# Xinglab/lr2rmats

Hardware: AMD Instinct MI355X
Metric: long-read alignments classified/sec; achieved HBM GB/s vs roofline (higher is better)
Workload: dtype int32

## Files before the change

lr2rmats_amd/csrc/l2r_engine.hip:

```cpp
#include <hip/hip_runtime.h>
#include <stdarg.h>
#include <stdio.h>
#include <stdlib.h>
#include <string.h>
#include <algorithm>
#include <initializer_list>
#include <string>
#include <type_traits>
#include <utility>
#include <vector>

#include "../../include/lr2rmats_hip.h"
#include "l2r_kernels.hip.h"
#include "l2r_window.hip.h"
#include "l2r_slab.hip.h"
#include "l2r_chunk.hip.h"
#include "l2r_tchunk.hip.h"
#include "l2r_filter.hip.h"
#include "l2r_fusion.hip.h"
#include "l2r_sj.hip.h"
#include "l2r_sort.hip.h"
#include "l2r_names.hip.h"
#include "l2r_gtf.hip.h"
#include "l2r_bed.hip.h"
#include "l2r_uniq.hip.h"
#include "l2r_plan.hip.h"
#include "l2r_tables.hip.h"
#include "l2r_nameorder.hip.h"
#include "l2r_gtforder.hip.h"
#include "l2r_bedplan.hip.h"

using namespace l2r;

static thread_local char g_err[1024] = "";

static int fail(int code, const char *fmt, ...)
{
    va_list ap;
    va_start(ap, fmt);
    vsnprintf(g_err, sizeof g_err, fmt, ap);
    va_end(ap);
    return code;
}

#define HIP_TRY(expr)                                                                                   \
    do {                                                                                                \
        hipError_t e_ = (expr);                                                                         \
        if (e_ != hipSuccess) return fail(-2, "[%s] %s: %s", __func__, #expr, hipGetErrorString(e_));   \
    } while (0)

template <typename T>
struct DevBuf {
    T *p = nullptr;
    size_t cap = 0;
    DevBuf() = default;
    DevBuf(const DevBuf &) = delete;
    DevBuf &operator=(const DevBuf &) = delete;
    ~DevBuf() { release(); }
    int ensure(size_t n)
    {
        if (n <= cap && p) return 0;
        if (p) { (void)hipFree(p); p = nullptr; cap = 0; }
        const size_t want = n ? n : 1;
        T *q = nullptr;
        const hipError_t e = hipMalloc((void **)&q, want * sizeof(T));
        if (e != hipSuccess) return fail(-2, "hipMalloc(%zu bytes): %s", want * sizeof(T), hipGetErrorString(e));
        p = q; cap = want;
        return 0;
    }
    void release() { if (p) (void)hipFree(p); p = nullptr; cap = 0; }
};

struct EventPair {
    hipEvent_t a = nullptr, b = nullptr;
    EventPair() = default;
    EventPair(const EventPair &) = delete;
    EventPair &operator=(const EventPair &) = delete;
    ~EventPair() { if (a) (void)hipEventDestroy(a); if (b) (void)hipEventDestroy(b); }
};

struct StageTimer {
    bool on = false, wait = false;
    hipEvent_t ev[2] = {nullptr, nullptr};
    StageTimer() = default;
    StageTimer(const StageTimer &) = delete;
    StageTimer &operator=(const StageTimer &) = delete;
    ~StageTimer() { for (int k = 0; k < 2; ++k) if (ev[k]) (void)hipEventDestroy(ev[k]); }
    int begin(bool on_, bool wait_)
    {
        on = on_; wait = wait_;
        for (int k = 0; k < 2 && on; ++k) if (!ev[k]) HIP_TRY(hipEventCreate(&ev[k]));
        return 0;
    }
    template <typename F> int launch(l2r_ctx *c, double *ms, F f);
};

enum class Pipeline { classic, slab, tile };

struct SjRowBuf {
    DevBuf<int32_t> col[6];
    size_t cap = 0;
    SjCols cols() const { return SjCols{col[0].p, col[1].p, col[2].p, col[3].p, col[4].p, col[5].p}; }
};
struct SjState {
    bool open = false, finished = false;
    bool over = false;
    SjPrm prm{3, 1};
    int32_t n_seq = 0;
    DevBuf<int64_t> seq_off; DevBuf<uint8_t> bases;
    SjRowBuf rows[2]; int cur = 0;
    int64_t n_rows = 0;
    int64_t compact_rows = (int64_t)1 << 24, compact_at = (int64_t)1 << 24;
    DevBuf<uint16_t> flag; DevBuf<int32_t> tid, pos; DevBuf<uint8_t> uniq; DevBuf<int64_t> cig_off; DevBuf<uint32_t> cig, cnt;
    DevBuf<uint32_t> hist12, tile_hist, head, word;
    DevBuf<uint8_t> strand[2], motif[2], anno[2]; int bcur = 0;
    DevBuf<int32_t> near_acc;
    double stats[32] = {0};
    StageTimer clk;
};
struct SjIntrons {
    DevBuf<int32_t> tx_tid, ex_start, ex_end; DevBuf<int64_t> tx_ex_off;
    SjState st;
};

struct SortState {
    DevBuf<uint16_t> flag; DevBuf<int32_t> tid, pos;
    DevBuf<uint64_t> key[2]; DevBuf<uint32_t> idx[2];
    DevBuf<uint32_t> hist, tile_hist, word;
    StageTimer clk;
    double stats[7] = {0};
};

struct NameState {
    DevBuf<uint64_t> blob, hkey;
    DevBuf<int64_t> off;
    DevBuf<uint32_t> head, head_pos, first_idx, sizes, order;
    DevBuf<uint32_t> word;
    StageTimer clk;
    double stats[11] = {0};
};

struct GtfState {
    DevBuf<uint4> text;
    DevBuf<uint32_t> tile_cnt, start;
    DevBuf<uint32_t> kept, tx, l_name_off, l_name_len, l_s, l_e;
    DevBuf<uint32_t> r_start, r_len, r_line, r_tx;
    DevBuf<uint32_t> t_name_off, t_name_len, t_s, t_e, head;
    DevBuf<uint32_t> h_off, h_len, rank;
    DevBuf<uint32_t> c, s, e, order1, order;
    DevBuf<uint32_t> word;
    std::vector<uint64_t> res_start; std::vector<uint32_t> res_len, res_line;
    StageTimer clk;
    double stats[17] = {0};
};

struct BedState {
    bool begun = false;
    l2r_bed_params prm{};
    std::vector<int64_t> h_ref_off; std::vector<uint8_t> h_ref_names;
    DevBuf<int64_t> ref_off; DevBuf<uint8_t> ref_names;
    DevBuf<uint16_t> flag; DevBuf<int32_t> tid, pos; DevBuf<uint8_t> mapq, names; DevBuf<int64_t> cig_off, name_off; DevBuf<uint32_t> cig;
    DevBuf<uint32_t> off, n_blocks, span, size_len;
    DevBuf<uint32_t> word;
    DevBuf<uint4> text;
    bool have_text = false, text_on_host = false;
    int64_t n_bytes = 0;
    std::vector<uint8_t> host_text;
    StageTimer clk;
    double stats[11] = {0};
};

struct UniqState {
    DevBuf<int32_t> tid, xs, xe; DevBuf<uint8_t> rev; DevBuf<int64_t> ex_off;
    DevBuf<UniqRec> rec; DevBuf<uint64_t> tile_max;
    DevBuf<uint32_t> head, first, len, word;
    DevBuf<int32_t> l_src, l_start, l_end, l_cov;
    DevBuf<int32_t> uniq_of, u_src, u_start, u_end, u_cov; DevBuf<uint8_t> merged;
    bool have = false, on_host = false;
    int64_t n = 0, n_unique = 0;
    UniqResult host;
    StageTimer clk;
    double stats[UQS_N] = {0};
};

struct RunFacts {
    bool known = false;
    uint32_t n_wide = 0;
    uint32_t n_chunk = 0;
    uint32_t n_rest = 0;
    uint32_t n_late = 0;
    uint32_t n_fb = 0;
    uint32_t n_wide_rest = 0;
    unsigned long long chunk_rest = 0;
    bool redo_empty = false;
};

struct l2r_ctx {
    int device = 0;
    hipStream_t stream = nullptr;
    hipStream_t side[2] = {nullptr, nullptr};
    hipEvent_t ev_fork = nullptr, ev_join[2] = {nullptr, nullptr};

    int fast_grid = 0;
    int n_cu = 256, wg_per_cu = 4;
    int ablate = 0;
    int64_t seg_max = SEG_MAX;
    Pipeline want_pipe = Pipeline::tile;
    bool pipeline_forced = false;
    bool wide_direct = true;
    bool chunk_direct = true;
    bool tile_split = true;
    bool side_on = true;
    bool env_tile_anyway = false, env_launch_all = false;
    bool check_stages = false;
    bool env_stamps = false;
    int64_t tile_resident = 0;
    bool tile_starved = false;
    int64_t n_lb_fallback = 0;

    l2r_params prm;
    std::string anno_cache_dir;
    int anno_cache_state = 0;
    unsigned want = L2R_WANT_RESULTS | L2R_WANT_ACCEPTED;
    bool one_shot_upload = false;

    bool sorted = true;
    int reads_per_tile = TILE_THREADS;
    int64_t n_tiles = 0, n_tiles256 = 0;
    bool wide_cigar = false;
    bool many_exon_reads = false;
    bool slab_ok = false;
    bool have_index = false;
    float index_ms = 0.0f;
    DevBuf<SlotRec> slot_rec;
    DevBuf<TileStat> tile_stat; std::vector<TileStat> h_tile_stat;
    DevBuf<TileStat> sup_stat;
    DevBuf<uint16_t> sum_nn;
    DevBuf<uint32_t> tile_sbase, s_pre, s_loc, s_pl, cig_off32, tile_rec, tile_total, tile_xbase, tile_span;
    DevBuf<int32_t> dense_start, dense_end;
    DevBuf<uint32_t> slab_row;
    DevBuf<TileWin> tw;
    DevBuf<TileWin64> tw64; DevBuf<uint32_t> wide_list, chunk_list, list_cnt, tile_flags;
    DevBuf<unsigned long long> ovf_cursor;
    DevBuf<unsigned long long> lb_tile, lb_blk, lb_sup;
    DevBuf<uint32_t> fb_list;
    DevBuf<uint32_t> rest_list;

    Pipeline pipe = Pipeline::classic;
    bool prev_run_tile = false;
    uint32_t lc_flip = 0;
    uint32_t lb_flip = 0;
    RunFacts facts;
    int64_t inexact_tiles = -1;
    int64_t n_tx = 0, n_anno_exon = 0;
    DevBuf<TxHdr> hdr;
    DevBuf<int2> anno_ex;
    DevBuf<int64_t> anno_key;
    DevBuf<SiteEnt> sk_st, sk_en;
    DevBuf<uint32_t> sd_st, sd_en, sr_st;
    DevBuf<int32_t> tid_base; int32_t n_tid_dir = 0;
    DevBuf<uint32_t> key_dir; DevBuf<int32_t> kb_base; int32_t n_tid_key = 0;
    DevBuf<int32_t> j0;
    int64_t n_compact = 0, n_wide = 0;
    std::vector<int64_t> h_anno_key_raw;
    std::vector<int64_t> h_anno_key_pm;
    int64_t n_sj = 0;
    DevBuf<int32_t> sj_tid, sj_don, sj_acc, sj_uniq, sj_multi;
    DevBuf<int64_t> sj_key;
    DevBuf<int32_t> sj_cbase, sj_dbase; DevBuf<uint32_t> sj_cdir, sj_ddir; DevBuf<int4> sj_row; int32_t sj_ntid = 0;
    std::vector<int64_t> h_sj_key_raw;
    std::vector<int64_t> h_sj_key_pm;
    int64_t n_reads = 0, n_cigar = 0, first_read = 0;
    DevBuf<int32_t> r_tid, r_pos;
    DevBuf<uint8_t> r_rev;
    DevBuf<int64_t> cig_off;
    DevBuf<uint32_t> cig;
    std::vector<int32_t> h_tid, h_pos;
    struct Stream {
        bool valid = false, sorted = true;
        int64_t next = 0;
        int64_t last_key = INT64_MIN;
        int64_t anno_cur = 0, sj_cur = 0;
        int64_t anno_cur_start = 0, sj_cur_start = 0;
        bool sj_pending = false;
    } seq;
    DevBuf<int32_t> win_start, sj_cursor;
    bool have_win = false;
    DevBuf<uint32_t> local, tile_base, ex_off, info, tile_acc, tile_acc_ex, tile_acc_at, tile_acc_ex_at, tile_chunk, tile_rchunk, totals;
    DevBuf<uint32_t> redo;
    DevBuf<uint8_t> order;
    DevBuf<TileDesc> desc;
    DevBuf<int2> walked;
    DevBuf<uint32_t> tile_first;
    DevBuf<TxHdr> win_hdr;
    DevBuf<int32_t> ex_start, ex_end, ref_tx;
    DevBuf<uint8_t> ex_flag;
    int64_t ex_cap = 0;
    DevBuf<AccRec> acc_rec;
    DevBuf<uint32_t> acc_ex_off;
    DevBuf<int32_t> acc_start, acc_end;
    DevBuf<uint8_t> acc_flag;
    bool ran = false;
    DevBuf<unsigned long long> stamps;
    uint32_t h_totals[3] = {0, 0, 0};
    bool totals_valid = false;
    SjState sj;
    SjIntrons sj_intr;
    double fusion_stats[5] = {0, 0, 0, 0, 0};
    StageTimer fusion_clk;
    SortState sort;
    NameState name;
    GtfState gtf;
    BedState bed;
    UniqState uniq;
};

template <typename F> int StageTimer::launch(l2r_ctx *c, double *ms, F f)
{
    if (on) HIP_TRY(hipEventRecord(ev[0], c->stream));
    f();
    HIP_TRY(hipGetLastError());
    if (on) {
        float t = 0.0f;
        HIP_TRY(hipEventRecord(ev[1], c->stream));
        HIP_TRY(hipEventSynchronize(ev[1]));
        HIP_TRY(hipEventElapsedTime(&t, ev[0], ev[1]));
        *ms += t;
    }
    if (wait) HIP_TRY(hipStreamSynchronize(c->stream));
    return 0;
}

static void forget_list_state(l2r_ctx *c)
{
    c->facts = RunFacts{};
    c->inexact_tiles = -1;
}

static bool lists_empty(const RunFacts &f) { return f.n_fb == 0u && f.n_wide == 0u && f.n_chunk == 0u && f.n_late == 0u; }
static bool lists_heavy(const l2r_ctx *c)
{
    const RunFacts &f = c->facts;
    return 2ull * ((unsigned long long)f.n_fb + (c->wide_direct ? f.n_wide_rest : f.n_wide) + f.chunk_rest) > (unsigned long long)c->n_tiles;
}
static bool list_runs(const l2r_ctx *c, unsigned long long n) { return !c->facts.known || n != 0ull || c->env_launch_all; }
static unsigned list_grid(const l2r_ctx *c, uint32_t n) { return c->facts.known ? std::max(n, 1u) : (unsigned)std::max<int64_t>(c->n_tiles, 1); }

static uint32_t *lc_this_run(const l2r_ctx *c) { return c->list_cnt.p + LC_WORDS * (c->lc_flip & 1u); }
static uint32_t *lc_next_run(const l2r_ctx *c) { return c->list_cnt.p + LC_WORDS * ((c->lc_flip & 1u) ^ 1u); }
static uint32_t *lc_last_run(const l2r_ctx *c) { return lc_next_run(c); }
static hipError_t lc_reset(l2r_ctx *c) { c->lc_flip = 0; return hipMemsetAsync(c->list_cnt.p, 0, 2 * LC_WORDS * sizeof(uint32_t), c->stream); }
static void end_of_run(l2r_ctx *c, bool tile) { if (tile) { c->lb_flip ^= 1u; c->lc_flip ^= 1u; } c->prev_run_tile = tile; }

static DevParams dev_params(const l2r_ctx *c)
{
    DevParams p;
    p.min_exon = c->prm.min_exon; p.min_intron = c->prm.min_intron; p.max_delet = c->prm.max_delet;
    p.ss_dis = c->prm.ss_dis; p.full_level = c->prm.full_level; p.use_multi = c->prm.use_multi;
    p.min_sj_cnt = c->prm.min_sj_cnt; p.split_trans = c->prm.split_trans; p.frac = c->prm.single_exon_ovlp_frac;
    p.n_tx = (int32_t)c->n_tx; p.n_sj = (int32_t)c->n_sj; p.reads_per_tile = c->reads_per_tile;
    p.ablate = c->ablate; p.want = (int32_t)c->want;
    if (c->n_sj > 0 && (c->ablate & (512 | 1024))) p.ablate |= 2;
    return p;
}

template <typename F> static void with_level(int level, F &&f)
{
    switch (level) {
    case 1: f(std::integral_constant<int, 1>()); break;
    case 2: f(std::integral_constant<int, 2>()); break;
    case 3: f(std::integral_constant<int, 3>()); break;
    case 4: f(std::integral_constant<int, 4>()); break;
    case 5: f(std::integral_constant<int, 5>()); break;
    default: f(std::integral_constant<int, 0>()); break;
    }
}
template <typename F> static void with_flag(bool on, F &&f)
{
    if (on) f(std::true_type());
    else f(std::false_type());
}

template <bool WIDE, bool EXACT>
static void launch_k_tile(const l2r_ctx *c, const DevParams &p, const SlabArgs &sa, unsigned grid, hipStream_t st)
{
    with_level(p.full_level, [&](auto L) { with_flag(p.ss_dis > 0, [&](auto D) { with_flag(!WIDE && (c->want & L2R_WANT_ACCEPTED), [&](auto A) {
        if constexpr (!(WIDE && A))
            hipLaunchKernelGGL(HIP_KERNEL_NAME(k_tile<L, A, D, WIDE, EXACT>), dim3(grid), dim3(TILE_THREADS), 0, st, sa, (const TileRec *)c->tile_rec.p, (const TileWin *)c->tw.p,
                               (const TileStat *)c->tile_stat.p, (const SlotRec *)c->slot_rec.p, c->tile_xbase.p);
    }); }); });
}

template <typename T> static int to_dev(l2r_ctx *c, DevBuf<T> &b, const T *src, size_t n)
{
    if (b.ensure(n ? n : 1)) return -2;
    if (n) HIP_TRY(hipMemcpyAsync(b.p, src, n * sizeof(T), hipMemcpyHostToDevice, c->stream));
    return 0;
}
template <typename T> static int put_dev(l2r_ctx *c, DevBuf<T> &b, const std::vector<T> &v) { return to_dev(c, b, v.data(), v.size()); }

extern "C" {

int l2r_abi_version(void) { return L2R_ABI_VERSION; }
const char *l2r_last_error(void) { return g_err; }

int l2r_device_count(void)
{
    int n = 0;
    if (hipGetDeviceCount(&n) != hipSuccess) return 0;
    return n;
}

l2r_ctx *l2r_create(int device)
{
    int n = 0;
    hipError_t e = hipGetDeviceCount(&n);
    if (e != hipSuccess || n <= 0) { fail(-1, "[l2r_create] no HIP device available (%s); this library has no CPU path", hipGetErrorString(e)); return nullptr; }
    if (device < 0 || device >= n) { fail(-1, "[l2r_create] device %d out of range (have %d)", device, n); return nullptr; }
    if ((e = hipSetDevice(device)) != hipSuccess) { fail(-2, "[l2r_create] hipSetDevice: %s", hipGetErrorString(e)); return nullptr; }
    l2r_ctx *c = new l2r_ctx();
    c->device = device;
    if ((e = hipStreamCreateWithFlags(&c->stream, hipStreamNonBlocking)) != hipSuccess) {
        fail(-2, "[l2r_create] hipStreamCreate: %s", hipGetErrorString(e)); delete c; return nullptr;
    }
    int prio_lo = 0, prio_hi = 0;
    (void)hipDeviceGetStreamPriorityRange(&prio_lo, &prio_hi);
    for (int k = 0; k < 2; ++k)
        if (((e = hipStreamCreateWithPriority(&c->side[k], hipStreamNonBlocking, prio_hi)) != hipSuccess &&
             ((void)hipGetLastError(), e = hipStreamCreateWithFlags(&c->side[k], hipStreamNonBlocking)) != hipSuccess) ||
            (e = hipEventCreateWithFlags(&c->ev_join[k], hipEventDisableTiming)) != hipSuccess) {
            fail(-2, "[l2r_create] side stream: %s", hipGetErrorString(e)); l2r_destroy(c); return nullptr;
        }
    if ((e = hipEventCreateWithFlags(&c->ev_fork, hipEventDisableTiming)) != hipSuccess) { fail(-2, "[l2r_create] hipEventCreate: %s", hipGetErrorString(e)); l2r_destroy(c); return nullptr; }
    c->prm = l2r_params{3, 3, 50, 0, 0x7fffffff, 5, 0, 0, 1, 0, 0.80f};
    {
        hipDeviceProp_t prop;
        if (hipGetDeviceProperties(&prop, device) == hipSuccess && prop.multiProcessorCount > 0) c->n_cu = prop.multiProcessorCount;
        const char *e = getenv("L2R_WG_PER_CU");
        if (e && atoi(e) > 0) c->wg_per_cu = atoi(e);
        e = getenv("L2R_FAST_GRID");
        if (e && atoi(e) > 0) c->fast_grid = atoi(e);
        e = getenv("L2R_ABLATE");
        c->ablate = e ? atoi(e) : 0;
        c->check_stages = getenv("L2R_CHECK") != nullptr;
        e = getenv("L2R_SEG_MAX");
        if (e && atoll(e) >= 0) c->seg_max = atoll(e);
        e = getenv("L2R_ANNO_CACHE");
        if (e && *e) c->anno_cache_dir = e;
        e = getenv("L2R_WIDE_DIRECT");
        if (e) c->wide_direct = atoi(e) != 0;
        c->env_tile_anyway = getenv("L2R_TILE_ANYWAY") != nullptr; c->env_launch_all = getenv("L2R_LAUNCH_ALL") != nullptr;
        e = getenv("L2R_CHUNK_DIRECT");
        if (e) c->chunk_direct = atoi(e) != 0;
        e = getenv("L2R_TILE_SPLIT");
        if (e) c->tile_split = atoi(e) != 0;
        e = getenv("L2R_SIDE");
        if (e) c->side_on = atoi(e) != 0;
        c->env_stamps = getenv("L2R_STAMPS") != nullptr;
        e = getenv("L2R_PIPELINE");
        if (e) { c->want_pipe = !strcmp(e, "classic") ? Pipeline::classic : !strcmp(e, "slab") ? Pipeline::slab : Pipeline::tile; c->pipeline_forced = true; }
        {
            int per_cu = 0;
            if (hipOccupancyMaxActiveBlocksPerMultiprocessor(&per_cu, k_tile<3, false, false, false>, TILE_THREADS, 0) != hipSuccess) { (void)hipGetLastError(); per_cu = 0; }
            c->tile_resident = (int64_t)per_cu * c->n_cu;
            if ((int64_t)per_cu * c->n_cu < 8 * (int64_t)TILE_GROUP + 1 || getenv("L2R_TILE_STARVED")) c->tile_starved = true;
        }
    }
    return c;
}

void l2r_destroy(l2r_ctx *c)
{
    if (!c) return;
    (void)hipSetDevice(c->device);
    for (int k = 0; k < 2; ++k) { if (c->side[k]) (void)hipStreamDestroy(c->side[k]); if (c->ev_join[k]) (void)hipEventDestroy(c->ev_join[k]); }
    if (c->ev_fork) (void)hipEventDestroy(c->ev_fork);
    if (c->stream) (void)hipStreamDestroy(c->stream);
    delete c;
}

void *l2r_stream(l2r_ctx *c) { return c ? (void *)c->stream : nullptr; }
float l2r_upload_index_ms(l2r_ctx *c) { return c ? c->index_ms : 0.0f; }
int l2r_hint_single_run(l2r_ctx *c, int on) { if (!c) return fail(-1, "[l2r_hint_single_run] null context"); c->one_shot_upload = on != 0; return 0; }

int l2r_set_outputs(l2r_ctx *c, unsigned want)
{
    if (!c) return fail(-1, "[l2r_set_outputs] null context");
    if (!(want & (L2R_WANT_RESULTS | L2R_WANT_ACCEPTED)) || (want & ~(unsigned)(L2R_WANT_RESULTS | L2R_WANT_ACCEPTED)))
        return fail(-1, "[l2r_set_outputs] want = %u: expected L2R_WANT_RESULTS and/or L2R_WANT_ACCEPTED", want);
    c->want = want;
    c->ran = false; forget_list_state(c);
    return 0;
}

int l2r_set_params(l2r_ctx *c, const l2r_params *prm)
{
    if (!c || !prm) return fail(-1, "[l2r_set_params] null argument");
    c->prm = *prm;
    c->ran = false; forget_list_state(c);
    return 0;
}

int l2r_set_annotation_cache(l2r_ctx *c, const char *dir)
{
    if (!c) return fail(-1, "[l2r_set_annotation_cache] null context");
    c->anno_cache_dir = dir ? dir : "";
    return 0;
}

int l2r_annotation_cache_state(l2r_ctx *c) { return c ? c->anno_cache_state : -1; }

int l2r_set_annotation(l2r_ctx *c, const l2r_annotation *a)
{
    if (!c || !a) return fail(-1, "[l2r_set_annotation] null argument");
    if (a->n_tx < 0 || a->n_tx > 0x7ffffff0LL || a->n_exon < 0 || a->n_exon > 0x7ffffff0LL) return fail(-1, "[l2r_set_annotation] size out of range");
    HIP_TRY(hipSetDevice(c->device));
    AnnoTables t;
    std::string msg;
    c->anno_cache_state = 0;
    const int state = anno_tables(a, c->anno_cache_dir, t, msg);
    if (state < 0) return fail(-1, "%s", msg.c_str());
    c->anno_cache_state = state;
    int rc = 0;
    if ((rc = put_dev(c, c->sk_st, t.st_ent)) || (rc = put_dev(c, c->sd_st, t.st_dir)) || (rc = put_dev(c, c->sr_st, t.st_rdir)) ||
        (rc = put_dev(c, c->sk_en, t.en_ent)) || (rc = put_dev(c, c->sd_en, t.en_dir)) || (rc = put_dev(c, c->tid_base, t.tid_base)) ||
        (rc = put_dev(c, c->key_dir, t.key_dir)) || (rc = put_dev(c, c->kb_base, t.kb_base)) || (rc = put_dev(c, c->hdr, t.hdr)) ||
        (rc = put_dev(c, c->anno_key, t.key)) || (rc = put_dev(c, c->anno_ex, t.ex))) return rc;
    HIP_TRY(hipStreamSynchronize(c->stream));
    c->h_anno_key_raw.swap(t.key_raw);
    c->h_anno_key_pm.swap(t.key);
    c->seq = l2r_ctx::Stream();
    c->n_compact = t.n_compact; c->n_wide = t.n_wide; c->n_tid_dir = t.n_tid_dir; c->n_tid_key = t.n_tid_key;
    c->n_tx = a->n_tx; c->n_anno_exon = a->n_exon;
    c->have_win = false; c->ran = false; forget_list_state(c);
    return 0;
}

int l2r_set_junctions(l2r_ctx *c, const l2r_junctions *s)
{
    if (!c) return fail(-1, "[l2r_set_junctions] null context");
    HIP_TRY(hipSetDevice(c->device));
    c->ran = false; forget_list_state(c);
    if (!s || s->n == 0) { c->n_sj = 0; c->h_sj_key_raw.clear(); c->h_sj_key_pm.clear(); c->seq = l2r_ctx::Stream(); return 0; }
    SjTables t;
    std::string msg;
    if (build_sj_tables(s, t, msg)) return fail(-1, "%s", msg.c_str());
    const size_t n = (size_t)s->n;
    int rc = 0;
    if ((rc = put_dev(c, c->sj_row, t.row)) || (rc = put_dev(c, c->sj_cbase, t.cbase)) || (rc = put_dev(c, c->sj_cdir, t.cdir)) ||
        (rc = put_dev(c, c->sj_dbase, t.dbase)) || (rc = put_dev(c, c->sj_ddir, t.ddir)) ||
        (rc = to_dev(c, c->sj_tid, s->tid, n)) || (rc = to_dev(c, c->sj_don, s->don, n)) || (rc = to_dev(c, c->sj_acc, s->acc, n)) ||
        (rc = to_dev(c, c->sj_uniq, s->uniq_c, n)) || (rc = to_dev(c, c->sj_multi, s->multi_c, n)) || (rc = put_dev(c, c->sj_key, t.key))) return rc;
    HIP_TRY(hipStreamSynchronize(c->stream));
    c->sj_ntid = t.n_tid;
    c->n_sj = s->n;
    c->h_sj_key_raw.swap(t.key_raw);
    c->h_sj_key_pm.swap(t.key);
    c->seq = l2r_ctx::Stream();
    return 0;
}

static int prepare_unsorted_windows(l2r_ctx *c);
static int finish_stream_sj_cursor(l2r_ctx *c);

static int stream_begin_upload(l2r_ctx *c, const l2r_reads *r)
{
    l2r_ctx::Stream &st = c->seq;
    const bool cont = st.valid && r->first_read_index > 0 && r->first_read_index == st.next;
    if (cont) { int rc = finish_stream_sj_cursor(c); if (rc) return rc; }
    else st = l2r_ctx::Stream();
    st.anno_cur_start = st.anno_cur; st.sj_cur_start = st.sj_cur;
    st.next = r->first_read_index + r->n_reads; st.valid = true;
    st.sj_pending = false;
    return 0;
}

static int stage_reads(l2r_ctx *c, const l2r_reads *r, const UploadPlan &pl)
{
    const int64_t N = r->n_reads;
    if (c->tile_first.ensure(pl.tile_first.size())) return -2;
    HIP_TRY(hipMemcpyAsync(c->tile_first.p, pl.tile_first.data(), pl.tile_first.size() * 4, hipMemcpyHostToDevice, c->stream));
    if (c->r_tid.ensure((size_t)N) || c->r_pos.ensure((size_t)N) || c->r_rev.ensure((size_t)N) ||
        c->cig_off.ensure((size_t)N + 1) || c->cig.ensure((size_t)r->n_cigar + 8)) return -2;
    if (N) {
        HIP_TRY(hipMemcpyAsync(c->r_tid.p, r->tid, (size_t)N * 4, hipMemcpyHostToDevice, c->stream));
        HIP_TRY(hipMemcpyAsync(c->r_pos.p, r->pos, (size_t)N * 4, hipMemcpyHostToDevice, c->stream));
        HIP_TRY(hipMemcpyAsync(c->r_rev.p, r->rev, (size_t)N, hipMemcpyHostToDevice, c->stream));
        HIP_TRY(hipMemcpyAsync(c->cig_off.p, r->cig_off, (size_t)(N + 1) * 8, hipMemcpyHostToDevice, c->stream));
        if (r->n_cigar) HIP_TRY(hipMemcpyAsync(c->cig.p, r->cig, (size_t)r->n_cigar * 4, hipMemcpyHostToDevice, c->stream));
    }
    return 0;
}

static int count_exon_bound(l2r_ctx *c, const l2r_reads *r, bool wide_cigar, size_t *exb)
{
    *exb = (size_t)r->n_cigar + (size_t)r->n_reads;
    if (!wide_cigar) return 0;
    if (c->totals.ensure(TOT_WORDS)) return -2;
    unsigned long long *d_cnt = reinterpret_cast<unsigned long long *>(c->totals.p);
    HIP_TRY(hipMemsetAsync(d_cnt, 0, 8, c->stream));
    hipLaunchKernelGGL(k_count_cut_ops, dim3(4096), dim3(TILE_THREADS), 0, c->stream, (const uint32_t *)c->cig.p, (int64_t)r->n_cigar, d_cnt);
    unsigned long long cuts = 0;
    HIP_TRY(hipMemcpyAsync(&cuts, d_cnt, 8, hipMemcpyDeviceToHost, c->stream));
    HIP_TRY(hipStreamSynchronize(c->stream));
    *exb = (size_t)cuts + (size_t)r->n_reads;
    return 0;
}

static int reserve_work(l2r_ctx *c, size_t n_reads, size_t exb)
{
    const size_t N = n_reads, T = (size_t)c->n_tiles;
    if (c->j0.ensure(N) || c->local.ensure(N + 1) || c->ex_off.ensure(N) || c->info.ensure(N) || c->ref_tx.ensure(N) ||
        c->redo.ensure(N) || c->order.ensure(N + TILE_THREADS) || c->desc.ensure(T) || c->win_hdr.ensure(T * WIN_TX) ||
        c->tile_base.ensure(T + 1) || c->tile_acc.ensure(T + 1) || c->tile_acc_ex.ensure(T + 1) ||
        c->tile_acc_at.ensure(T + 2) || c->tile_acc_ex_at.ensure(T + 2) ||
        c->totals.ensure(TOT_WORDS) || c->tile_chunk.ensure(T + 1) || c->tile_rchunk.ensure(T + 1) || c->ex_start.ensure(exb) || c->ex_end.ensure(exb) || c->ex_flag.ensure(exb) ||
        c->acc_rec.ensure(N) || c->acc_ex_off.ensure(N) ||
        c->acc_start.ensure(exb) || c->acc_end.ensure(exb) || c->acc_flag.ensure(exb) || (c->wide_cigar && c->walked.ensure((T + 1) * LDS_EXON_CAP))) return -2;
    c->ex_cap = (int64_t)exb;
    return 0;
}

static int stage_slab(l2r_ctx *c, size_t n_reads, const UploadPlan &pl)
{
    const size_t N = n_reads, T = (size_t)pl.n_tiles;
    if (c->tw64.ensure(T + 1) || c->wide_list.ensure(2 * (T + 1)) || c->chunk_list.ensure(2 * (T + 1)) || c->list_cnt.ensure(2 * LC_WORDS) || c->tile_flags.ensure(T + 8) ||
        c->lb_tile.ensure(T + 64) || c->lb_blk.ensure(T / LB_BLK + 64) || c->lb_sup.ensure(2 * ((T >> LB_SUP_SHIFT) + 64)) || c->fb_list.ensure(T + 1) || c->rest_list.ensure(T + 1) || c->tile_stat.ensure(T + 1) || c->sup_stat.ensure((T >> LB_SUP_SHIFT) + 2) ||
        (!c->wide_cigar && c->slot_rec.ensure((T + 1) * TILE_THREADS))) return -2;
    HIP_TRY(hipMemsetAsync(c->lb_sup.p, 0, 2 * ((T >> LB_SUP_SHIFT) + 64) * 8, c->stream)); c->lb_flip = 0;
    HIP_TRY(lc_reset(c)); c->prev_run_tile = false;
    if (c->tile_sbase.ensure(T + 1) || c->ovf_cursor.ensure(1) || c->tw.ensure(T + 1) || c->tile_total.ensure(T + 2) || c->tile_xbase.ensure(T + 2) || c->tile_span.ensure(12 * (T + 1)) ||
        c->s_pre.ensure(N + 1) || c->s_loc.ensure(N + 1) ||
        c->slab_row.ensure((size_t)pl.slab_total + 4) ||
        c->dense_start.ensure((size_t)pl.dense_rows + 1) || c->dense_end.ensure((size_t)pl.dense_rows + 1)) return -2;
    HIP_TRY(hipMemsetAsync(c->ovf_cursor.p, 0, 8, c->stream));
    HIP_TRY(hipMemcpyAsync(c->tile_sbase.p, pl.sbase.data(), (T + 1) * 4, hipMemcpyHostToDevice, c->stream));
    if (c->tile_rec.ensure(8 * (T + 1)) || c->cig_off32.ensure(N + 2) || c->s_pl.ensure(N + 1)) return -2;
    HIP_TRY(hipMemcpyAsync(c->tile_rec.p, pl.rec.data(), pl.rec.size() * sizeof(TileRec), hipMemcpyHostToDevice, c->stream));
    HIP_TRY(hipMemcpyAsync(c->cig_off32.p, pl.off32.data(), pl.off32.size() * 4, hipMemcpyHostToDevice, c->stream));
    return 0;
}

static int make_tile_index(l2r_ctx *c, const l2r_reads *r, const UploadPlan &pl)
{
    const size_t N = (size_t)r->n_reads, T = (size_t)pl.n_tiles;
    const bool summaries = r->cig_summary != nullptr;
    c->h_tile_stat = pl.tile_stat;
    c->index_ms = 0.0f; c->have_index = pl.have_index;
    if (!pl.have_index) return 0;
    EventPair ev;
    HIP_TRY(hipEventCreate(&ev.a)); HIP_TRY(hipEventCreate(&ev.b));
    if (summaries) {
        if (c->sum_nn.ensure(N + 1)) return -2;
        HIP_TRY(hipMemcpyAsync(c->sum_nn.p, pl.nn.data(), N * 2, hipMemcpyHostToDevice, c->stream));
        HIP_TRY(hipMemcpyAsync(c->tile_stat.p, c->h_tile_stat.data(), T * sizeof(TileStat), hipMemcpyHostToDevice, c->stream));
    }
    const unsigned gi = (unsigned)std::min<size_t>(T, 8192);
    HIP_TRY(hipEventRecord(ev.a, c->stream));
    with_flag(summaries, [&](auto S) {
        hipLaunchKernelGGL(HIP_KERNEL_NAME(k_tile_index<S>), dim3(gi), dim3(TILE_THREADS), 0, c->stream, (TileRec *)c->tile_rec.p, c->tile_stat.p, c->slot_rec.p, (uint32_t)T,
                           (const uint32_t *)c->cig_off32.p, (const int32_t *)c->r_pos.p, (const uint8_t *)c->r_rev.p, (const uint32_t *)c->cig.p, S ? (const uint16_t *)c->sum_nn.p : (const uint16_t *)nullptr);
    });
    HIP_TRY(hipEventRecord(ev.b, c->stream));
    if (!summaries) {
        HIP_TRY(hipMemcpyAsync(c->h_tile_stat.data(), c->tile_stat.p, T * sizeof(TileStat), hipMemcpyDeviceToHost, c->stream));
        HIP_TRY(hipStreamSynchronize(c->stream));
    }
    HIP_TRY(hipEventSynchronize(ev.b));
    HIP_TRY(hipEventElapsedTime(&c->index_ms, ev.a, ev.b));
    return 0;
}

int l2r_upload_reads(l2r_ctx *c, const l2r_reads *r)
{
    if (!c || !r) return fail(-1, "[l2r_upload_reads] null argument");
    if (r->n_reads < 0 || r->n_cigar < 0) return fail(-1, "[l2r_upload_reads] negative size");
    if ((uint64_t)r->n_cigar + (uint64_t)r->n_reads >= 0xfffffff0ULL)
        return fail(-1, "[l2r_upload_reads] shard too large for 32-bit exon offsets (%lld ops + %lld reads); split it", (long long)r->n_cigar, (long long)r->n_reads);
    HIP_TRY(hipSetDevice(c->device));
    const int64_t N = r->n_reads;
    UploadPlan pl;
    std::vector<TileStat> sup;
    struct Drain { hipStream_t s; ~Drain() { (void)hipStreamSynchronize(s); } } drain{c->stream};
    std::string msg;
    if (int rc = plan_check_reads(*r, pl, msg)) return fail(rc, "%s", msg.c_str());

    if (int rc = stream_begin_upload(c, r)) return rc;

    PlanOpts po;
    po.min_intron = c->prm.min_intron; po.max_delet = c->prm.max_delet;
    po.want_slab = c->want_pipe != Pipeline::classic;
    po.want_index = c->want_pipe == Pipeline::tile && !(c->one_shot_upload && !c->env_tile_anyway && !c->pipeline_forced);
    po.stream_sorted = c->seq.sorted; po.last_key = c->seq.last_key;
    plan_tiles(*r, po, pl);
    c->seq.sorted = pl.sorted; c->seq.last_key = pl.last_key;
    const bool sorted = pl.sorted;
    c->sorted = sorted; c->have_win = false;
    if (!sorted || c->n_sj > 0) { c->h_tid.assign(r->tid, r->tid + N); c->h_pos.assign(r->pos, r->pos + N); }
    else { c->h_tid.clear(); c->h_pos.clear(); }
    c->wide_cigar = pl.wide_cigar; c->many_exon_reads = pl.many_exon_reads;
    c->reads_per_tile = pl.reads_per_tile; c->n_tiles = pl.n_tiles; c->n_tiles256 = pl.n_tiles256;

    if (int rc = stage_reads(c, r, pl)) return rc;
    size_t exb = 0;
    if (int rc = count_exon_bound(c, r, pl.wide_cigar, &exb)) return rc;
    if (int rc = reserve_work(c, (size_t)N, exb)) return rc;

    plan_slab(*r, exb, pl);
    c->slab_ok = pl.slab_ok; c->pipe = Pipeline::classic;
    if (pl.slab_ok) {
        if (int rc = stage_slab(c, (size_t)N, pl)) return rc;
        if (int rc = make_tile_index(c, r, pl)) return rc;
        sup = plan_sup_stat(pl, c->h_tile_stat);
        HIP_TRY(hipMemcpyAsync(c->sup_stat.p, sup.data(), sup.size() * sizeof(TileStat), hipMemcpyHostToDevice, c->stream));
    }
    if (c->env_stamps && !c->stamps.p) {
        if (c->stamps.ensure(1024 * 8 + 16)) return -2;
        HIP_TRY(hipMemsetAsync(c->stamps.p, 0, (1024 * 8 + 16) * 8, c->stream));
    }
    HIP_TRY(hipStreamSynchronize(c->stream));

    c->n_reads = N; c->n_cigar = r->n_cigar; c->first_read = r->first_read_index;
    c->ran = false; c->totals_valid = false; forget_list_state(c);
    if (sorted) {
        if (N) c->seq.anno_cur = std::max(c->seq.anno_cur, cursor_after(c->h_anno_key_pm, r->tid[N - 1], r->pos[N - 1]));
        c->seq.sj_pending = c->n_sj > 0;
    } else {
        int rc = prepare_unsorted_windows(c);
        if (rc) return rc;
    }
    return 0;
}

static int finish_stream_sj_cursor(l2r_ctx *c)
{
    l2r_ctx::Stream &st = c->seq;
    if (!st.sj_pending || !c->ran || c->n_sj == 0 || c->n_reads == 0) { st.sj_pending = false; return 0; }
    const int64_t N = c->n_reads;
    std::vector<uint32_t> info((size_t)N);
    HIP_TRY(hipMemcpyAsync(info.data(), c->info.p, (size_t)N * 4, hipMemcpyDeviceToHost, c->stream));
    HIP_TRY(hipStreamSynchronize(c->stream));
    for (int64_t i = N - 1; i >= 0; --i) {
        if ((info[(size_t)i] & (I_FULL | I_KNOWN | I_KSITE)) != (I_FULL | I_KSITE)) continue;
        st.sj_cur = std::max(st.sj_cur, cursor_after(c->h_sj_key_pm, c->h_tid[(size_t)i], c->h_pos[(size_t)i]));
        break;
    }
    st.sj_pending = false;
    return 0;
}

static int prepare_unsorted_windows(l2r_ctx *c)
{
    if (c->sorted || c->have_win) return 0;
    const int64_t N = c->n_reads;
    std::vector<int32_t> w((size_t)N);
    c->seq.anno_cur = cursor_replay(c->h_anno_key_raw, c->seq.anno_cur_start, c->h_tid.data(), c->h_pos.data(), N, w.data(), [](int64_t) { return true; });
    if (c->win_start.ensure((size_t)N)) return -2;
    if (N) HIP_TRY(hipMemcpyAsync(c->win_start.p, w.data(), (size_t)N * 4, hipMemcpyHostToDevice, c->stream));
    HIP_TRY(hipStreamSynchronize(c->stream));
    c->have_win = true;
    return 0;
}

static int prepare_unsorted_sj_cursor(l2r_ctx *c)
{
    const int64_t N = c->n_reads;
    std::vector<uint32_t> info((size_t)N);
    if (N) HIP_TRY(hipMemcpyAsync(info.data(), c->info.p, (size_t)N * 4, hipMemcpyDeviceToHost, c->stream));
    HIP_TRY(hipStreamSynchronize(c->stream));
    std::vector<int32_t> cur_v((size_t)N);
    c->seq.sj_cur = cursor_replay(c->h_sj_key_raw, c->seq.sj_cur_start, c->h_tid.data(), c->h_pos.data(), N, cur_v.data(),
                                  [&](int64_t i) { return (info[(size_t)i] & (I_FULL | I_KNOWN | I_KSITE)) == (I_FULL | I_KSITE); });
    if (c->sj_cursor.ensure((size_t)N)) return -2;
    if (N) HIP_TRY(hipMemcpyAsync(c->sj_cursor.p, cur_v.data(), (size_t)N * 4, hipMemcpyHostToDevice, c->stream));
    HIP_TRY(hipStreamSynchronize(c->stream));
    return 0;
}

enum { ST_PASS_A = 0, ST_SCAN1, ST_FAST, ST_GENERIC, ST_SJ, ST_SCAN2, ST_GATHER, ST_N };

static Pipeline choose_pipeline(l2r_ctx *c, const DevParams &p)
{
    if (!(c->slab_ok && p.min_intron >= 0 && p.min_intron < (1 << 28) && p.max_delet >= -1 && p.max_delet < (1 << 28) - 1 &&
          (!c->wide_cigar || p.min_exon >= 1)))
        return Pipeline::classic;
    if (c->want_pipe != Pipeline::tile || c->wide_cigar || p.min_exon < 1 || !(c->have_index || c->n_tiles == 0) || c->tile_starved)
        return Pipeline::slab;
    if (c->inexact_tiles < 0) {
        int64_t inexact = 0;
        for (const TileStat &st : c->h_tile_stat) inexact += tile_exact(st, p.min_exon, p.min_intron, p.max_delet) ? 0 : 1;
        c->inexact_tiles = inexact;
    }
    if (c->inexact_tiles * 50 > c->n_tiles + 800 && !c->env_tile_anyway) return Pipeline::slab;
    if (c->facts.known && lists_heavy(c) && !c->env_tile_anyway) return Pipeline::slab;
    return Pipeline::tile;
}

static const char *const stage_name[ST_N + 1] = {"(start)", "pass A / order", "scan / walk", "classification", "generic", "junction check", "accepted scan", "accepted gather"};
#define MARK(i) do { if (ev) HIP_TRY(hipEventRecord(ev[i], c->stream)); \
        if (c->check_stages) { const hipError_t e_ = hipStreamSynchronize(c->stream); \
            if (e_ != hipSuccess) return fail(-2, "[launch_all] device error behind stage \"%s\": %s", stage_name[i], hipGetErrorString(e_)); } } while (0)

static FastArgs fast_args(const l2r_ctx *c, const DevParams &p, const SiteTabs &tabs, const int32_t *j0)
{
    FastArgs fa;
    fa.n_reads = c->n_reads; fa.r_tid = c->r_tid.p; fa.r_pos = c->r_pos.p; fa.r_rev = c->r_rev.p; fa.cig_off = c->cig_off.p; fa.cig = c->cig.p;
    fa.walked = c->walked.p; fa.local = c->local.p; fa.order = c->order.p; fa.tile_base = c->tile_base.p; fa.j0 = j0; fa.desc = c->desc.p; fa.win_hdr = c->win_hdr.p;
    fa.hdr = c->hdr.p; fa.st = tabs.st; fa.en = tabs.en;
    fa.ex_off = c->ex_off.p; fa.ex_start = c->ex_start.p; fa.ex_end = c->ex_end.p; fa.ex_flag = c->ex_flag.p; fa.info = c->info.p; fa.ref_tx = c->ref_tx.p;
    fa.tile_acc = c->tile_acc.p; fa.tile_acc_ex = c->tile_acc_ex.p; fa.redo_count = c->totals.p + TOT_REDO; fa.redo = c->redo.p;
    fa.tile_chunk = c->tile_chunk.p; fa.tile_rchunk = c->tile_rchunk.p; fa.chunk_cursor = (unsigned long long *)(c->totals.p + TOT_CHUNK_CURSOR);
    fa.acc_start = c->acc_start.p; fa.acc_end = c->acc_end.p; fa.acc_flag = c->acc_flag.p; fa.acc_rec = (AccRec *)c->acc_rec.p; fa.acc_ex_off = c->acc_ex_off.p; fa.first_read = c->first_read;
    fa.stamps = c->stamps.p; fa.p = p;
    return fa;
}

static bool split_wait_free(const l2r_ctx *c) { return c->inexact_tiles == 0 && !(c->ablate & 256); }
static uint32_t split_mode(const l2r_ctx *c)
{
    if (!c->tile_split || !c->rest_list.p) return SPLIT_OFF;
    const uint32_t fits = (uint32_t)std::min<int64_t>((int64_t)c->n_cu * 4, c->tile_resident / 2);
    if (c->facts.known) return c->facts.n_rest <= fits ? SPLIT_ON : SPLIT_OFF;
    return split_wait_free(c) ? SPLIT_ON : SPLIT_LIST;
}

static SlabArgs slab_args(const l2r_ctx *c, const FastArgs &fa, const CursorDir &cd, bool tile)
{
    SlabArgs sa;
    sa.g.f = fa; sa.g.cd = cd; sa.g.tid_base = c->tid_base.p; sa.g.n_tid_dir = c->n_tid_dir; sa.g.tile_total = c->tile_total.p;
    sa.tile_sbase = c->tile_sbase.p; sa.slab_row = c->slab_row.p;
    sa.dense_start = c->dense_start.p; sa.dense_end = c->dense_end.p; sa.ovf_cursor = c->ovf_cursor.p;
    sa.pl = c->s_pl.p; sa.pre_x = c->s_pre.p; sa.loc_x = c->s_loc.p; sa.cig_off32 = c->cig_off32.p; sa.tw = c->tw.p; sa.span = (TileSpan *)c->tile_span.p;
    sa.n_tiles = (uint32_t)c->n_tiles;
    sa.tw64 = (c->ablate & 4) ? nullptr : c->tw64.p;
    sa.chunk_on = (c->ablate & 32) ? 0u : 1u;
    sa.wide_list = c->wide_list.p; sa.chunk_list = c->chunk_list.p; sa.list_cnt = c->list_cnt.p; sa.list_cnt_next = nullptr; sa.tile_flags = c->tile_flags.p;
    if (tile) { sa.list_cnt = lc_this_run(c); sa.list_cnt_next = lc_next_run(c); }
    {   const size_t sup_words = (size_t)(c->n_tiles >> LB_SUP_SHIFT) + 64;
        sa.lb_sup = c->lb_sup.p ? c->lb_sup.p + (c->lb_flip ? sup_words : 0) : nullptr;
        sa.lb_sup_next = c->lb_sup.p ? c->lb_sup.p + (c->lb_flip ? 0 : sup_words) : nullptr;
        sa.n_sup = (uint32_t)(c->n_tiles >> LB_SUP_SHIFT) + 1u; }
    sa.lb_tile = c->lb_tile.p; sa.lb_blk = c->lb_blk.p; sa.lb_err = c->totals.p + TOT_LB_ERR; sa.fb_list = c->fb_list.p; sa.exon_total = c->totals.p + TOT_EXONS; sa.tile_stat = c->tile_stat.p; sa.sup_stat = c->sup_stat.p;
    sa.sj = SjDir{CursorDir{c->sj_key.p, c->sj_cdir.p, c->sj_cbase.p, c->sj_ntid, (int32_t)c->n_sj}, c->sj_ddir.p, c->sj_dbase.p, c->sj_ntid, c->sj_row.p};
    sa.has_wide_keys = c->n_wide > 0 ? 1u : 0u;
    sa.wide_direct_on = (tile && c->wide_direct && c->tw64.p && !(c->ablate & 4)) ? 1u : 0u;
    sa.chunk_direct_on = (tile && c->chunk_direct && sa.chunk_on) ? 1u : 0u;
    sa.rest_list = c->rest_list.p;
    sa.split_on = tile ? split_mode(c) : SPLIT_OFF;
    return sa;
}

static void launch_probe(const l2r_ctx *c, const DevParams &p, const SlabArgs &sa, bool list, bool acc, unsigned grid)
{
    with_level(p.full_level, [&](auto L) { with_flag(p.ss_dis > 0, [&](auto D) { with_flag(list, [&](auto LIST) { with_flag(acc && !list, [&](auto A) {
        if constexpr (!(A && LIST))
            hipLaunchKernelGGL(HIP_KERNEL_NAME(k_probe_slab<L, A, D, LIST>), dim3(grid), dim3(TILE_THREADS), 0, c->stream, sa, (const TileSpan *)c->tile_span.p,
                               (const TileWin *)c->tw.p, (const uint32_t *)c->tile_xbase.p, (const uint32_t *)c->fb_list.p);
    }); }); }); });
}

static void launch_tile_chunk(const l2r_ctx *c, const DevParams &p, const SlabArgs &sa, unsigned grid, uint32_t late, hipStream_t s)
{
    with_level(p.full_level, [&](auto L) {
        hipLaunchKernelGGL(HIP_KERNEL_NAME(k_tile_chunk<L>), dim3(grid), dim3(TILE_THREADS), 0, s, sa, (const TileRec *)c->tile_rec.p, (const TileWin *)c->tw.p,
                           (const TileStat *)c->tile_stat.p, (const SlotRec *)c->slot_rec.p, c->tile_xbase.p, late);
    });
}

static int launch_classic(l2r_ctx *c, hipEvent_t *ev, const DevParams &p, const FastArgs &fa, const CursorDir &cd, const SiteTabs &tabs)
{
    hipStream_t s = c->stream;
    const unsigned gt = (unsigned)(c->n_tiles ? c->n_tiles : 1);
    with_flag(c->wide_cigar, [&](auto W) {
        hipLaunchKernelGGL(HIP_KERNEL_NAME(k_pass_a<W>), dim3(gt), dim3(TILE_THREADS), W ? pass_a_dynamic_lds(c->reads_per_tile) : 0, s, c->n_reads, c->r_tid.p, c->r_pos.p,
                           c->cig_off.p, c->cig.p, cd, tabs, p, (c->sorted ? (const int32_t *)nullptr : (const int32_t *)c->win_start.p), c->j0.p, c->local.p, c->order.p,
                           c->tile_base.p, c->desc.p, c->totals.p + TOT_REDO, (const TxHdr *)c->hdr.p, c->win_hdr.p, (const uint32_t *)c->tile_first.p, c->walked.p);
    });
    MARK(ST_SCAN1);
    {
        ScanJobs jobs = {}; jobs.job[0] = ScanJob{c->tile_base.p, c->n_tiles, c->totals.p + TOT_EXONS}; jobs.job[1] = jobs.job[0];
        hipLaunchKernelGGL(k_scan_u32, dim3(1), dim3(1024), 0, s, jobs);
    }
    MARK(ST_FAST);
    unsigned gp = (unsigned)std::min<int64_t>(c->n_tiles ? c->n_tiles : 1, (int64_t)c->n_cu * c->wg_per_cu);
    if (c->fast_grid > 0) gp = (unsigned)std::min<int64_t>(gp, c->fast_grid);
    with_level(p.full_level, [&](auto L) { with_flag(c->wide_cigar, [&](auto W) {
        hipLaunchKernelGGL(HIP_KERNEL_NAME(k_classify_fast<L, W>), dim3(gp), dim3(TILE_THREADS), 0, s, fa, c->n_tiles, (const TileDesc *)c->desc.p,
                           (const uint32_t *)c->tile_base.p, (const int64_t *)c->cig_off.p, (const uint8_t *)c->order.p, (const uint32_t *)c->tile_first.p);
    }); });
    return 0;
}

static int launch_slab(l2r_ctx *c, hipEvent_t *ev, const DevParams &p, const SlabArgs &sa)
{
    hipStream_t s = c->stream;
    const unsigned gx = 8u * (unsigned)std::max<int64_t>((c->n_tiles + 7) / 8, 1);
    if (c->wide_cigar)
        hipLaunchKernelGGL(k_walk_slab_long, dim3(gx), dim3(TILE_THREADS), pass_a_dynamic_lds(c->reads_per_tile), s, sa, (const TileRec *)c->tile_rec.p);
    else
        with_flag(p.min_exon < 1, [&](auto E) { hipLaunchKernelGGL(HIP_KERNEL_NAME(k_walk_slab<E>), dim3(gx), dim3(TILE_THREADS), 0, s, sa, (const TileRec *)c->tile_rec.p); });
    MARK(ST_SCAN1);
    {
        const DescribeScan job{c->tile_total.p, c->tile_xbase.p, c->totals.p + TOT_EXONS, c->n_tiles};
        unsigned n_scan = (unsigned)std::max<int64_t>((c->n_tiles + DESCRIBE_SEG - 1) / DESCRIBE_SEG, 1);
        if (c->n_tiles > c->seg_max) {
            HIP_TRY(hipMemcpyAsync(c->tile_xbase.p, c->tile_total.p, (size_t)c->n_tiles * 4, hipMemcpyDeviceToDevice, s));
            ScanJobs jobs = {}; jobs.job[0] = ScanJob{c->tile_xbase.p, c->n_tiles, c->totals.p + TOT_EXONS}; jobs.job[1] = jobs.job[0];
            hipLaunchKernelGGL(k_scan_u32, dim3(1), dim3(1024), 0, s, jobs);
            n_scan = 0;
        }
        const unsigned gd = n_scan + (unsigned)std::max<int64_t>((c->n_tiles + DESCRIBE_TILES - 1) / DESCRIBE_TILES, 1);
        hipLaunchKernelGGL(HIP_KERNEL_NAME(k_describe_scan<false>), dim3(gd), dim3(TILE_THREADS), 0, s, sa, job, (uint32_t)n_scan, (const TileRec *)nullptr);
    }
    MARK(ST_FAST);
    launch_probe(c, p, sa, false, (c->want & L2R_WANT_ACCEPTED) && c->n_sj == 0, gx);
    return 0;
}

static int launch_tile(l2r_ctx *c, hipEvent_t *ev, const DevParams &p, const SlabArgs &sa, bool skip_lists)
{
    hipStream_t s = c->stream;
    const RunFacts &f = c->facts;
    const DescribeScan job{c->tile_total.p, c->tile_xbase.p, c->totals.p + TOT_EXONS, c->n_tiles};
    const unsigned gd = (unsigned)std::max<int64_t>((c->n_tiles + DESCRIBE_TILES - 1) / DESCRIBE_TILES, 1);
    hipLaunchKernelGGL(HIP_KERNEL_NAME(k_describe_scan<true>), dim3(gd), dim3(TILE_THREADS), 0, s, sa, job, 0u, (const TileRec *)c->tile_rec.p);
    MARK(ST_SCAN1);
    const bool split = sa.split_on == SPLIT_ON;
    const bool rest_launch = split && list_runs(c, f.n_rest);
    const bool wide_launch = !skip_lists && sa.wide_direct_on && list_runs(c, f.n_wide);
    const bool chunk_launch = !skip_lists && sa.chunk_direct_on && list_runs(c, f.n_chunk);
    const bool beside = c->side_on && !ev && !c->check_stages;
    const bool rest_side = rest_launch && beside && split_wait_free(c);
    const bool wide_side = wide_launch && beside, chunk_side = chunk_launch && beside;
    const bool side0 = rest_side || wide_side, side1 = chunk_side;
    const unsigned gf = fused_grid(c->n_tiles), gr = list_grid(c, f.n_rest), gwd = list_grid(c, f.n_wide), gcd = list_grid(c, f.n_chunk);
    if (rest_launch && !rest_side) launch_k_tile<false, false>(c, p, sa, gr, s);
    if (side0 || side1) HIP_TRY(hipEventRecord(c->ev_fork, s));
    if (side0) HIP_TRY(hipStreamWaitEvent(c->side[0], c->ev_fork, 0));
    if (rest_side) launch_k_tile<false, false>(c, p, sa, gr, c->side[0]);
    if (wide_launch) launch_k_tile<true, false>(c, p, sa, gwd, wide_side ? c->side[0] : s);
    if (side0) HIP_TRY(hipEventRecord(c->ev_join[0], c->side[0]));
    if (side1) {
        HIP_TRY(hipStreamWaitEvent(c->side[1], c->ev_fork, 0));
        launch_tile_chunk(c, p, sa, gcd, 0u, c->side[1]);
        HIP_TRY(hipEventRecord(c->ev_join[1], c->side[1]));
    }
    if (split) launch_k_tile<false, true>(c, p, sa, gf, s);
    else launch_k_tile<false, false>(c, p, sa, gf, s);
    MARK(ST_FAST);
    if (chunk_launch && !chunk_side) launch_tile_chunk(c, p, sa, gcd, 0u, s);
    if (side0) HIP_TRY(hipStreamWaitEvent(s, c->ev_join[0], 0));
    if (side1) HIP_TRY(hipStreamWaitEvent(s, c->ev_join[1], 0));
    const unsigned gl = (unsigned)std::min<int64_t>(c->n_tiles ? c->n_tiles : 1, (int64_t)c->n_cu * 2);
    if (!skip_lists && list_runs(c, f.n_fb)) launch_probe(c, p, sa, true, false, gl);
    return 0;
}

static void launch_lists(l2r_ctx *c, const DevParams &p, const SlabArgs &sa, bool tile, bool skip_lists)
{
    if (skip_lists) return;
    hipStream_t s = c->stream;
    const RunFacts &f = c->facts;
    if (!tile || list_runs(c, f.n_wide_rest)) {
        const WideArgs wa{c->tw64.p};
        const unsigned gw = (unsigned)std::min<int64_t>(c->n_tiles ? c->n_tiles : 1, (int64_t)c->n_cu * 5);
        with_level(p.full_level, [&](auto L) {
            hipLaunchKernelGGL(HIP_KERNEL_NAME(k_probe_slab_wide<L>), dim3(gw), dim3(TILE_THREADS), 0, s, sa, wa, (const uint32_t *)c->tile_first.p, (const int32_t *)c->r_pos.p,
                               (const uint32_t *)c->tile_sbase.p, (const TileWin *)c->tw.p, (const uint32_t *)c->tile_xbase.p, (const TileStat *)(tile ? c->tile_stat.p : nullptr));
        });
    }
    if (sa.chunk_direct_on && list_runs(c, f.n_late)) {
        launch_tile_chunk(c, p, sa, list_grid(c, f.n_late), 1u, s);
    }
    if (sa.chunk_on && (!tile || list_runs(c, f.chunk_rest))) {
        const unsigned gc = (unsigned)std::min<int64_t>(c->n_tiles ? c->n_tiles : 1, (int64_t)c->n_cu * 4);
        with_level(p.full_level, [&](auto L) {
            hipLaunchKernelGGL(HIP_KERNEL_NAME(k_probe_slab_chunked<L>), dim3(gc), dim3(TILE_THREADS), 0, s, sa, (const uint32_t *)c->tile_first.p, (const int32_t *)c->r_pos.p,
                               (const uint32_t *)c->tile_sbase.p, (const TileWin *)c->tw.p, (const uint32_t *)c->tile_xbase.p);
        });
    }
}

static int launch_tail(l2r_ctx *c, hipEvent_t *ev, const DevParams &p, const CursorDir &cd, const int32_t *j0)
{
    hipStream_t s = c->stream;
    const bool tile = c->pipe == Pipeline::tile;
    const unsigned gt = (unsigned)(c->n_tiles ? c->n_tiles : 1), g256 = (unsigned)(c->n_tiles256 ? c->n_tiles256 : 1);
    MARK(ST_GENERIC);
    const bool sj_left = c->n_sj > 0 && (c->ablate & (512 | 1024)) != 0;
    const bool nothing_left = tile && c->facts.known && c->facts.redo_empty && (lists_empty(c->facts) || c->n_sj == 0) && !c->env_launch_all && !sj_left;
    end_of_run(c, tile);
    if (!nothing_left) {
        const unsigned gg = (unsigned)std::min<int64_t>(c->n_tiles ? c->n_tiles * 4 : 1, 4096);
        hipLaunchKernelGGL(k_classify_generic, dim3(gg), dim3(TILE_THREADS), 0, s, c->totals.p + TOT_REDO, c->redo.p, c->r_tid.p, c->r_rev.p,
                           (c->pipe != Pipeline::classic ? (const int32_t *)nullptr : j0),
                           c->hdr.p, c->anno_ex.p, p, c->ex_off.p, c->ex_start.p, c->ex_end.p, c->ex_flag.p, c->info.p, c->ref_tx.p,
                           c->tile_acc.p, c->tile_acc_ex.p, (const uint32_t *)c->tile_first.p, (int)c->n_tiles, cd);
    }
    MARK(ST_SJ);
    if (c->n_sj > 0 && !nothing_left) {
        if (!c->sorted) { int rc = prepare_unsorted_sj_cursor(c); if (rc) return rc; }
        hipLaunchKernelGGL(k_validate_sj, dim3(g256), dim3(TILE_THREADS), 0, s, c->n_reads, c->r_tid.p, c->ex_off.p, c->ex_start.p, c->ex_end.p, c->ex_flag.p,
                           c->sj_key.p, (c->sorted ? (const int32_t *)nullptr : c->sj_cursor.p), c->sj_tid.p, c->sj_don.p, c->sj_acc.p,
                           c->sj_uniq.p, c->sj_multi.p, p, c->info.p,
                           SjDir{CursorDir{c->sj_key.p, c->sj_cdir.p, c->sj_cbase.p, c->sj_ntid, (int32_t)c->n_sj}, c->sj_ddir.p, c->sj_dbase.p, c->sj_ntid, c->sj_row.p});
    }
    if ((c->n_sj > 0 || c->pipe != Pipeline::classic) && (c->want & L2R_WANT_ACCEPTED)) {
        hipLaunchKernelGGL(k_count_accepted, dim3((gt + 3u) / 4u), dim3(TILE_THREADS), 0, s, (const uint32_t *)c->tile_first.p, c->info.p, (const uint32_t *)c->tile_chunk.p, c->tile_acc.p, c->tile_acc_ex.p, (uint32_t)c->n_tiles);
    }
    MARK(ST_SCAN2);
    if (c->want & L2R_WANT_ACCEPTED) {
        if (c->n_tiles <= c->seg_max) {
            const unsigned n_seg = (unsigned)std::max<int64_t>((c->n_tiles + SEG_COUNT - 1) / SEG_COUNT, 1);
            hipLaunchKernelGGL(k_scan_segments, dim3(2u * n_seg), dim3(TILE_THREADS), 0, s, SegScan{c->tile_acc.p, c->tile_acc_at.p, c->totals.p + TOT_ACCEPTED, c->n_tiles},
                               SegScan{c->tile_acc_ex.p, c->tile_acc_ex_at.p, c->totals.p + TOT_ACCEPTED_EXONS, c->n_tiles}, (uint32_t)n_seg);
        } else {
            HIP_TRY(hipMemcpyAsync(c->tile_acc_at.p, c->tile_acc.p, (size_t)c->n_tiles * 4, hipMemcpyDeviceToDevice, s));
            HIP_TRY(hipMemcpyAsync(c->tile_acc_ex_at.p, c->tile_acc_ex.p, (size_t)c->n_tiles * 4, hipMemcpyDeviceToDevice, s));
            ScanJobs jobs = {}; jobs.job[0] = ScanJob{c->tile_acc_at.p, c->n_tiles, c->totals.p + TOT_ACCEPTED}; jobs.job[1] = ScanJob{c->tile_acc_ex_at.p, c->n_tiles, c->totals.p + TOT_ACCEPTED_EXONS};
            hipLaunchKernelGGL(k_scan_u32, dim3(2), dim3(1024), 0, s, jobs);
        }
    }
    MARK(ST_GATHER);
    if (c->want & L2R_WANT_ACCEPTED)
        hipLaunchKernelGGL(k_gather_accepted, dim3((gt + GATHER_TILES - 1) / GATHER_TILES), dim3(TILE_THREADS), 0, s, (const uint32_t *)c->tile_first.p, c->first_read, c->info.p, c->ref_tx.p, c->ex_off.p,
                           c->ex_start.p, c->ex_end.p, c->ex_flag.p, c->tile_acc_at.p, c->tile_acc_ex_at.p, c->tile_chunk.p, c->tile_rchunk.p, c->totals.p + TOT_CHUNK_CURSOR,
                           c->acc_rec.p, c->acc_ex_off.p, c->acc_start.p, c->acc_end.p, c->acc_flag.p, (uint32_t)c->n_tiles);
    MARK(ST_N);
    return 0;
}

static int launch_all(l2r_ctx *c, hipEvent_t *ev )
{
    const DevParams p = dev_params(c);
    MARK(ST_PASS_A);
    c->pipe = choose_pipeline(c, p);
    const int32_t *j0 = c->sorted ? (const int32_t *)c->j0.p : (const int32_t *)c->win_start.p;
    const CursorDir cd{c->anno_key.p, c->key_dir.p, c->kb_base.p, c->n_tid_key, (int32_t)c->n_tx};
    const SiteTabs tabs{{c->sk_st.p, c->sd_st.p, c->sr_st.p}, {c->sk_en.p, c->sd_en.p, nullptr}, c->tid_base.p, c->n_tid_dir};
    const FastArgs fa = fast_args(c, p, tabs, j0);
    int rc = 0;
    if (c->pipe == Pipeline::classic) rc = launch_classic(c, ev, p, fa, cd, tabs);
    else {
        const bool tile = c->pipe == Pipeline::tile;
        if (tile && !c->prev_run_tile) HIP_TRY(lc_reset(c));
        const SlabArgs sa = slab_args(c, fa, cd, tile);
        const bool skip_lists = tile && c->facts.known && lists_empty(c->facts) && !c->env_launch_all;
        rc = tile ? launch_tile(c, ev, p, sa, skip_lists) : launch_slab(c, ev, p, sa);
        if (!rc) launch_lists(c, p, sa, tile, skip_lists);
    }
    if (!rc) rc = launch_tail(c, ev, p, cd, j0);
    if (rc) return rc;
    HIP_TRY(hipGetLastError());
    return 0;
}
#undef MARK

int l2r_debug_stamps(l2r_ctx *c, unsigned long long *out, int n)
{
    if (!c || !out) return fail(-1, "[l2r_debug_stamps] null argument");
    if (!c->stamps.p) { for (int i = 0; i < n; ++i) out[i] = 0; return 0; }
    std::vector<unsigned long long> h(1024 * 8 + 16);
    HIP_TRY(hipMemcpyAsync(h.data(), c->stamps.p, h.size() * 8, hipMemcpyDeviceToHost, c->stream));
    HIP_TRY(hipMemsetAsync(c->stamps.p, 0, h.size() * 8, c->stream));
    HIP_TRY(hipStreamSynchronize(c->stream));
    for (int i = 0; i < n; ++i) out[i] = 0;
    for (size_t k = 0; k < 1024 * 8; ++k) if ((int)(k & 7) < n) out[k & 7] += h[k];
    for (int i = 8; i < n && i < 16; ++i) out[i] = h[1024 * 8 + (i - 8)];
    return 0;
}

int l2r_debug_tile_times(l2r_ctx *c, uint32_t *out, int64_t n_tiles)
{
    if (!c || !out) return fail(-1, "[l2r_debug_tile_times] null argument");
    if (c->pipe != Pipeline::tile || !c->ran || n_tiles > c->n_tiles) return fail(-1, "[l2r_debug_tile_times] no run of the one-kernel tile path to report");
    HIP_TRY(hipSetDevice(c->device));
    const uint32_t *src[4] = {c->tile_total.p, c->tile_acc.p, c->tile_acc_ex.p, c->tile_flags.p};
    std::vector<uint32_t> h((size_t)n_tiles);
    for (int k = 0; k < 4; ++k) {
        HIP_TRY(hipMemcpyAsync(h.data(), src[k], (size_t)n_tiles * 4, hipMemcpyDeviceToHost, c->stream));
        HIP_TRY(hipStreamSynchronize(c->stream));
        for (int64_t i = 0; i < n_tiles; ++i) out[4 * i + k] = h[(size_t)i];
    }
    return 0;
}

int l2r_debug_counters(l2r_ctx *c, long long *out, int n)
{
    if (!c || !out || n < 4) return fail(-1, "[l2r_debug_counters] bad argument");
    HIP_TRY(hipSetDevice(c->device));
    uint32_t redo = 0;
    if (c->totals.p) { HIP_TRY(hipMemcpyAsync(&redo, c->totals.p + TOT_REDO, 4, hipMemcpyDeviceToHost, c->stream)); HIP_TRY(hipStreamSynchronize(c->stream)); }
    out[0] = redo; out[1] = c->n_wide; out[2] = c->n_compact; out[3] = c->n_tiles;
    if (n >= 12) for (int k = 0; k < 8; ++k) out[4 + k] = 0;
    if (n >= 13) out[12] = 0;
    for (int k = 16; k < std::min(n, 29); ++k) out[k] = 0;
    if (n >= 14) out[13] = c->n_lb_fallback;
    if (n >= 16) {
        out[14] = 0; out[15] = 0;
        if (c->pipe == Pipeline::tile && c->ran && c->list_cnt.p) {
            uint32_t lc[LC_WORDS];
            HIP_TRY(hipMemcpyAsync(lc, lc_last_run(c), sizeof lc, hipMemcpyDeviceToHost, c->stream));
            HIP_TRY(hipStreamSynchronize(c->stream));
            out[14] = lc[LC_DECLINED]; out[15] = lc[LC_LATE];
            if (n >= 29) out[28] = lc[LC_REST];
        }
    }
    if (n >= 12 && c->pipe != Pipeline::classic && c->ran && c->tw.p && c->n_tiles > 0) {
        std::vector<TileWin> w((size_t)c->n_tiles);
        HIP_TRY(hipMemcpyAsync(w.data(), c->tw.p, w.size() * sizeof(TileWin), hipMemcpyDeviceToHost, c->stream));
        HIP_TRY(hipStreamSynchronize(c->stream));
        for (const TileWin &t : w) {
            if (n >= 27) {
                out[24] = std::max<long long>(out[24], t.d.st_nk); out[25] = std::max<long long>(out[25], t.d.en_nk);
                if (t.d.flags & TD_CDIRECT) out[26]++;
                if (n >= 29 && c->pipe == Pipeline::tile && (t.d.flags & TD_XDIRECT)) out[27]++;
            }
            if (n >= 24) {
                const uint32_t why = (t.d.flags >> 8) & 7u;
                if ((t.d.flags & TD_CHUNK) || (!(t.d.flags & (TD_FAST | TD_WIDE)) && (why == 4u || why == 3u))) {
                    out[16 + (t.d.en_nk <= 256u ? 0 : t.d.en_nk <= 512u ? 1 : t.d.en_nk <= 768u ? 2 : t.d.en_nk <= 1024u ? 3 : 4)]++;
                    if (t.d.st_nk > 128u) out[21]++;
                    if (t.d.st_nk > 256u) out[22]++;
                    out[23]++;
                }
            }
            out[4 + ((t.d.flags >> 8) & 7u)]++;
            if (n >= 13 && (t.d.flags & TD_WIDE) && !(t.d.flags & TD_CHUNK)) out[12]++;
        }
    } else if (n >= 12 && c->pipe == Pipeline::classic && c->desc.p && c->n_tiles > 0) {
        std::vector<TileDesc> d((size_t)c->n_tiles);
        HIP_TRY(hipMemcpyAsync(d.data(), c->desc.p, d.size() * sizeof(TileDesc), hipMemcpyDeviceToHost, c->stream));
        HIP_TRY(hipStreamSynchronize(c->stream));
        for (const TileDesc &t : d) {
            out[4 + ((t.flags >> 8) & 7u)]++;
            if (n >= 27) { out[24] = std::max<long long>(out[24], t.st_nk); out[25] = std::max<long long>(out[25], t.en_nk); }
        }
    }
    return 0;
}

const char *l2r_stage_kernel(l2r_ctx *c, int stage)
{
    if (!c || stage < 0 || stage >= L2R_N_STAGES) return "";
    static const char *const classic[L2R_N_STAGES] = {"k_pass_a", "k_scan_u32 (tile sums)", "k_classify_fast", "k_classify_generic",
                                                      "k_validate_sj", "k_scan_accepted (k_scan_u32 of the accepted counts)", "k_gather_accepted", ""};
    if (stage >= 3 || c->pipe == Pipeline::classic) return classic[stage];
    if (c->pipe == Pipeline::tile) return stage == 0 ? "k_describe_scan (tile descriptors + tile lists; first kernel of the run)" : stage == 1 ? "k_tile (walk + probes + write-out, one workgroup per tile)" : "k_probe_slab (tiles k_tile left in slab form) (+ k_tile_chunk + k_probe_slab_wide + k_probe_slab_chunked)";
    return stage == 0 ? (c->wide_cigar ? "k_walk_slab_long" : "k_walk_slab") : stage == 1 ? "k_describe_scan (tile descriptors + scan of the exon counts + tile lists)" : "k_probe_slab (+ k_probe_slab_wide + k_probe_slab_chunked)";
}

int l2r_run(l2r_ctx *c)
{
    if (!c) return fail(-1, "[l2r_run] null context");
    HIP_TRY(hipSetDevice(c->device));
    int rc = prepare_unsorted_windows(c);
    if (rc) return rc;
    if ((rc = launch_all(c, nullptr))) return rc;
    c->ran = true; c->totals_valid = false;
    return 0;
}

static int fetch_run_facts(l2r_ctx *c)
{
    uint32_t lc[LC_WORDS];
    HIP_TRY(hipMemcpyAsync(lc, lc_last_run(c), sizeof lc, hipMemcpyDeviceToHost, c->stream));
    HIP_TRY(hipStreamSynchronize(c->stream));
    uint32_t redo_n = 1u;
    HIP_TRY(hipMemcpyAsync(&redo_n, c->totals.p + TOT_REDO, 4, hipMemcpyDeviceToHost, c->stream));
    HIP_TRY(hipStreamSynchronize(c->stream));
    RunFacts &f = c->facts;
    f.n_wide = lc[LC_WIDE]; f.n_chunk = lc[LC_CHUNK]; f.n_rest = lc[LC_REST]; f.n_late = lc[LC_LATE];
    f.n_fb = lc[LC_FB]; f.n_wide_rest = lc[LC_WIDE_REST];
    const bool tchunk = c->chunk_direct && !(c->ablate & 32);
    f.chunk_rest = tchunk ? (unsigned long long)lc[LC_DECLINED] + lc[LC_DECLINED_LATE] : (unsigned long long)lc[LC_LATE] + lc[LC_CHUNK];
    f.redo_empty = redo_n == 0u;
    f.known = true;
    return 0;
}

int l2r_sync(l2r_ctx *c)
{
    if (!c) return fail(-1, "[l2r_sync] null context");
    HIP_TRY(hipSetDevice(c->device));
    HIP_TRY(hipStreamSynchronize(c->stream));
    if (c->ran && c->pipe == Pipeline::tile && c->totals.p) {
        uint32_t lb = 0u;
        HIP_TRY(hipMemcpyAsync(&lb, c->totals.p + TOT_LB_ERR, 4, hipMemcpyDeviceToHost, c->stream));
        HIP_TRY(hipStreamSynchronize(c->stream));
        if (lb != 0u) {
            c->tile_starved = true; c->n_lb_fallback++;
            forget_list_state(c); c->totals_valid = false;
            int rc = launch_all(c, nullptr);
            if (rc) return rc;
            HIP_TRY(hipStreamSynchronize(c->stream));
            snprintf(g_err, sizeof g_err, "[l2r_sync] note: k_tile's look-back starved; the run was done again on the slab pipeline (this context keeps to it)");
        }
    }
    if (c->ran && c->pipe == Pipeline::tile && !c->facts.known && c->list_cnt.p) return fetch_run_facts(c);
    return 0;
}

static int fetch_totals(l2r_ctx *c)
{
    if (!c->ran) return fail(-1, "no completed run on this context");
    if (c->totals_valid) return 0;
    uint32_t dev[TOT_WORDS];
    HIP_TRY(hipMemcpyAsync(dev, c->totals.p, sizeof dev, hipMemcpyDeviceToHost, c->stream));
    HIP_TRY(hipStreamSynchronize(c->stream));
    if (c->pipe == Pipeline::tile && dev[TOT_LB_ERR] != 0u) return fail(-2, "[l2r] k_tile: a tile waited in vain for the exon counts of the tiles in front of it and l2r_sync was not called behind the run (it does the run again on the slab pipeline)");
    c->h_totals[0] = dev[TOT_EXONS]; c->h_totals[1] = dev[TOT_ACCEPTED] + dev[TOT_CHUNK_CURSOR + 1]; c->h_totals[2] = dev[TOT_ACCEPTED_EXONS] + dev[TOT_CHUNK_CURSOR];
    if (!(c->want & L2R_WANT_ACCEPTED)) c->h_totals[1] = c->h_totals[2] = 0;
    c->totals_valid = true;
    return 0;
}

int l2r_run_timed(l2r_ctx *c, int iters, l2r_timing *out)
{
    if (!c || !out || iters <= 0) return fail(-1, "[l2r_run_timed] bad argument");
    HIP_TRY(hipSetDevice(c->device));
    int rc = prepare_unsorted_windows(c);
    if (rc) return rc;
    memset(out, 0, sizeof *out);
    struct Events {
        hipEvent_t e[ST_N + 3]; int n = 0;
        ~Events() { for (int i = 0; i < n; ++i) (void)hipEventDestroy(e[i]); }
    } evs;
    for (int i = 0; i < ST_N + 3; ++i) { HIP_TRY(hipEventCreate(&evs.e[i])); evs.n = i + 1; }
    hipEvent_t t0 = evs.e[ST_N + 1], t1 = evs.e[ST_N + 2], *ev = evs.e;
    HIP_TRY(hipEventRecord(t0, c->stream));
    for (int it = 0; it < iters; ++it) { rc = launch_all(c, nullptr); if (rc) return rc; }
    HIP_TRY(hipEventRecord(t1, c->stream));
    HIP_TRY(hipEventSynchronize(t1));
    float ms = 0; HIP_TRY(hipEventElapsedTime(&ms, t0, t1));
    out->total_ms = ms / (float)iters;
    for (int it = 0; it < iters; ++it) {
        rc = launch_all(c, ev); if (rc) return rc;
        HIP_TRY(hipEventSynchronize(ev[ST_N]));
        for (int i = 0; i < ST_N; ++i) { float d = 0; HIP_TRY(hipEventElapsedTime(&d, ev[i], ev[i + 1])); out->stage_ms[i] += d / (float)iters; }
    }
    out->iters = iters;
    c->ran = true; c->totals_valid = false;
    return 0;
}

int l2r_result_sizes(l2r_ctx *c, int64_t *n_reads, int64_t *n_exons, int64_t *n_acc, int64_t *n_acc_ex)
{
    if (!c) return fail(-1, "[l2r_result_sizes] null context");
    HIP_TRY(hipSetDevice(c->device));
    int rc = fetch_totals(c);
    if (rc) return rc;
    if (n_reads) *n_reads = c->n_reads;
    if (n_exons) *n_exons = c->h_totals[0];
    if (n_acc) *n_acc = c->h_totals[1];
    if (n_acc_ex) *n_acc_ex = c->h_totals[2];
    return 0;
}

int l2r_download(l2r_ctx *c, l2r_result *res)
{
    if (!c || !res) return fail(-1, "[l2r_download] null argument");
    HIP_TRY(hipSetDevice(c->device));
    int rc = fetch_totals(c);
    if (rc) return rc;
    const int64_t N = c->n_reads, X = c->h_totals[0];
    if (res->n_reads < N || res->ex_cap < X) return fail(-3, "[l2r_download] buffers too small: need %lld reads, %lld exons", (long long)N, (long long)X);
    std::vector<uint32_t> off((size_t)N);
    if (N) {
        HIP_TRY(hipMemcpyAsync(off.data(), c->ex_off.p, (size_t)N * 4, hipMemcpyDeviceToHost, c->stream));
        HIP_TRY(hipMemcpyAsync(res->info, c->info.p, (size_t)N * 4, hipMemcpyDeviceToHost, c->stream));
        HIP_TRY(hipMemcpyAsync(res->ref_tx, c->ref_tx.p, (size_t)N * 4, hipMemcpyDeviceToHost, c->stream));
    }
    if (X) {
        HIP_TRY(hipMemcpyAsync(res->ex_start, c->ex_start.p, (size_t)X * 4, hipMemcpyDeviceToHost, c->stream));
        HIP_TRY(hipMemcpyAsync(res->ex_end, c->ex_end.p, (size_t)X * 4, hipMemcpyDeviceToHost, c->stream));
        HIP_TRY(hipMemcpyAsync(res->ex_flag, c->ex_flag.p, (size_t)X, hipMemcpyDeviceToHost, c->stream));
    }
    HIP_TRY(hipStreamSynchronize(c->stream));
    {
        int64_t at = 0;
        for (int64_t i = 0; i < N; ++i) {
            if ((int64_t)off[(size_t)i] != at) return fail(-5, "[l2r_download] exon offsets are not the running sum of the exon counts at read %lld (%u, expected %lld)", (long long)i, off[(size_t)i], (long long)at);
            res->ex_off[i] = at; at += (int64_t)(res->info[i] >> 8);
        }
        if (at != X) return fail(-5, "[l2r_download] exon counts (%lld) do not add up to the exon total (%lld)", (long long)at, (long long)X);
    }
    res->ex_off[N] = X;
    res->n_reads = N; res->n_exons = X;
    return 0;
}

static int order_accepted(const AccRec *rec, const uint32_t *off, std::vector<uint32_t> starts, const int32_t *xs, const int32_t *xe, const uint8_t *xf,
                          int64_t M, int64_t X, l2r_accepted *a, int64_t &at_r, int64_t &at)
{
    if (!M) return 0;
    const int64_t r_end = at_r + M, x_base = at;
    starts.push_back(0u);
    std::sort(starts.begin(), starts.end());
    starts.erase(std::unique(starts.begin(), starts.end()), starts.end());
    while (!starts.empty() && (int64_t)starts.back() >= M) starts.pop_back();
    std::vector<std::pair<uint64_t, std::pair<uint32_t, uint32_t>>> chunks;
    for (size_t k = 0; k < starts.size(); ++k) {
        const uint32_t from = starts[k], to = k + 1 < starts.size() ? starts[k + 1] : (uint32_t)M;
        chunks.push_back({((uint64_t)rec[from].read_hi << 32) | rec[from].read_lo, {from, to}});
    }
    std::sort(chunks.begin(), chunks.end());
    for (const auto &ch : chunks) {
        for (uint32_t i = ch.second.first; i < ch.second.second; ++i) {
            const int64_t n = (int64_t)(rec[i].info >> 8), from = off[i];
            if (from + n > X || at - x_base + n > X || at_r >= r_end) return fail(-5, "[l2r_download_accepted] inconsistent accepted list");
            memcpy(&a->rec[at_r], &rec[i], sizeof(AccRec));
            a->ex_off[at_r] = at;
            memcpy(a->ex_start + at, xs + from, (size_t)n * 4);
            memcpy(a->ex_end + at, xe + from, (size_t)n * 4);
            memcpy(a->ex_flag + at, xf + from, (size_t)n);
            at += n; ++at_r;
        }
    }
    if (at_r != r_end) return fail(-5, "[l2r_download_accepted] inconsistent accepted list (%lld of %lld records)", (long long)(at_r - (r_end - M)), (long long)M);
    return 0;
}

int l2r_download_accepted(l2r_ctx *c, l2r_accepted *a)
{
    if (!c || !a) return fail(-1, "[l2r_download_accepted] null argument");
    HIP_TRY(hipSetDevice(c->device));
    if (!(c->want & L2R_WANT_ACCEPTED)) return fail(-1, "[l2r_download_accepted] the accepted list was not requested (l2r_set_outputs)");
    int rc = fetch_totals(c);
    if (rc) return rc;
    const int64_t M = c->h_totals[1], X = c->h_totals[2];
    if (a->n_reads < M || a->ex_cap < X) return fail(-3, "[l2r_download_accepted] buffers too small: need %lld records, %lld exons", (long long)M, (long long)X);
    std::vector<AccRec> rec((size_t)M);
    std::vector<uint32_t> off((size_t)M), starts((size_t)c->n_tiles);
    std::vector<int32_t> xs((size_t)X), xe((size_t)X);
    std::vector<uint8_t> xf((size_t)X);
    if (M) {
        HIP_TRY(hipMemcpyAsync(rec.data(), c->acc_rec.p, (size_t)M * sizeof(AccRec), hipMemcpyDeviceToHost, c->stream));
        HIP_TRY(hipMemcpyAsync(off.data(), c->acc_ex_off.p, (size_t)M * 4, hipMemcpyDeviceToHost, c->stream));
        HIP_TRY(hipMemcpyAsync(starts.data(), c->tile_rchunk.p, (size_t)c->n_tiles * 4, hipMemcpyDeviceToHost, c->stream));
    }
    if (X) {
        HIP_TRY(hipMemcpyAsync(xs.data(), c->acc_start.p, (size_t)X * 4, hipMemcpyDeviceToHost, c->stream));
        HIP_TRY(hipMemcpyAsync(xe.data(), c->acc_end.p, (size_t)X * 4, hipMemcpyDeviceToHost, c->stream));
        HIP_TRY(hipMemcpyAsync(xf.data(), c->acc_flag.p, (size_t)X, hipMemcpyDeviceToHost, c->stream));
    }
    HIP_TRY(hipStreamSynchronize(c->stream));
    int64_t at_r = 0, at = 0;
    rc = order_accepted(rec.data(), off.data(), starts, xs.data(), xe.data(), xf.data(), M, X, a, at_r, at);
    if (rc) return rc;
    a->ex_off[M] = at;
    a->n_reads = M; a->n_exons = X;
    return 0;
}

int l2r_device_view_get(l2r_ctx *c, l2r_device_view *v)
{
    if (!c || !v) return fail(-1, "[l2r_device_view_get] null argument");
    HIP_TRY(hipSetDevice(c->device));
    int rc = fetch_totals(c);
    if (rc) return rc;
    v->n_reads = c->n_reads; v->n_exons = c->h_totals[0]; v->n_accepted = c->h_totals[1]; v->n_accepted_exons = c->h_totals[2];
    v->ex_off = nullptr; v->ex_start = nullptr; v->ex_end = nullptr; v->ex_flag = nullptr;
    if (c->want & L2R_WANT_RESULTS) { v->ex_off = c->ex_off.p; v->ex_start = c->ex_start.p; v->ex_end = c->ex_end.p; v->ex_flag = c->ex_flag.p; }
    v->info = c->info.p; v->ref_tx = c->ref_tx.p;
    v->acc_rec = (const l2r_accepted_read *)c->acc_rec.p; v->acc_ex_off = c->acc_ex_off.p;
    v->acc_ex_start = c->acc_start.p; v->acc_ex_end = c->acc_end.p; v->acc_ex_flag = c->acc_flag.p;
    return 0;
}

int l2r_classify(l2r_ctx *c, const l2r_reads *reads, l2r_result *res)
{
    if (!c) return fail(-1, "[l2r_classify] null context");
    const bool was = c->one_shot_upload;
    c->one_shot_upload = true;
    int rc = l2r_upload_reads(c, reads);
    c->one_shot_upload = was;
    if (rc) return rc;
    if ((rc = l2r_run(c))) return rc;
    if ((rc = l2r_sync(c))) return rc;
    return l2r_download(c, res);
}

extern "C++" {
static bool env_on(const char *name) { const char *e = getenv(name); return e && atoi(e) != 0; }

static int stats_out(const double *src, int have, double *out, int n, const char *who)
{
    if (!src || !out || n < 0) return fail(-1, "[%s] bad argument", who);
    for (int k = 0; k < n; ++k) out[k] = k < have ? src[k] : 0.0;
    return 0;
}

enum { FUS_WAVE = 0, FUS_K_SEG, FUS_K_SELECT, FUS_K_FILTER_SCORE, FUS_K_FILTER_SELECT, FUS_N };

static int fusion_begin(l2r_ctx *c, int slot)
{
    c->fusion_stats[slot] = 0;
    return c->fusion_clk.begin(env_on("L2R_FUSION_TIMING"), false);
}
// ... 1253 lines not shown
```

Baseline: 23.09 billion.

## Plan tile-pipeline launches from front counts read back mid-run

Adds a launch planner that builds the kernel launch sequence up front. On the first run it copies list counts to pinned host memory right after the main tile kernel is queued, waits on an event, and then sizes the rest/wide/chunk list launches to the real counts instead of full-tile grids. Lists that turn out empty are skipped. This is meant to remove oversized or empty list kernels on uncached runs. The cost is a host sync in the middle of the pipeline and more complex planning logic with a consistency check.

```diff
diff --git a/lr2rmats_amd/csrc/l2r_engine.hip b/lr2rmats_amd/csrc/l2r_engine.hip
--- a/lr2rmats_amd/csrc/l2r_engine.hip
+++ b/lr2rmats_amd/csrc/l2r_engine.hip
@@ -29,6 +29,7 @@
 #include "l2r_nameorder.hip.h"
 #include "l2r_gtforder.hip.h"
 #include "l2r_bedplan.hip.h"
+#include "l2r_launchplan.hip.h"
 
 using namespace l2r;
 
@@ -183,23 +184,13 @@
     double stats[UQS_N] = {0};
 };
 
-struct RunFacts {
-    bool known = false;
-    uint32_t n_wide = 0;
-    uint32_t n_chunk = 0;
-    uint32_t n_rest = 0;
-    uint32_t n_late = 0;
-    uint32_t n_fb = 0;
-    uint32_t n_wide_rest = 0;
-    unsigned long long chunk_rest = 0;
-    bool redo_empty = false;
-};
-
 struct l2r_ctx {
     int device = 0;
     hipStream_t stream = nullptr;
     hipStream_t side[2] = {nullptr, nullptr};
     hipEvent_t ev_fork = nullptr, ev_join[2] = {nullptr, nullptr};
+    hipEvent_t ev_front = nullptr;
+    uint32_t *h_front = nullptr;
 
     int fast_grid = 0;
     int n_cu = 256, wg_per_cu = 4;
@@ -212,6 +203,7 @@
     bool tile_split = true;
     bool side_on = true;
     bool env_tile_anyway = false, env_launch_all = false;
+    bool front_on = true;
     bool check_stages = false;
     bool env_stamps = false;
     int64_t tile_resident = 0;
@@ -251,6 +243,10 @@
     uint32_t lc_flip = 0;
     uint32_t lb_flip = 0;
     RunFacts facts;
+    FrontCounts front;
+    LaunchPlan plan; size_t plan_at = 0;
+    int64_t n_launches = 0, n_workgroups = 0;
+    int front_used = FRONT_NONE;
     int64_t inexact_tiles = -1;
     int64_t n_tx = 0, n_anno_exon = 0;
     DevBuf<TxHdr> hdr;
@@ -334,18 +330,15 @@
 static void forget_list_state(l2r_ctx *c)
 {
     c->facts = RunFacts{};
+    c->front = FrontCounts{};
     c->inexact_tiles = -1;
 }
 
-static bool lists_empty(const RunFacts &f) { return f.n_fb == 0u && f.n_wide == 0u && f.n_chunk == 0u && f.n_late == 0u; }
 static bool lists_heavy(const l2r_ctx *c)
 {
     const RunFacts &f = c->facts;
     return 2ull * ((unsigned long long)f.n_fb + (c->wide_direct ? f.n_wide_rest : f.n_wide) + f.chunk_rest) > (unsigned long long)c->n_tiles;
 }
-static bool list_runs(const l2r_ctx *c, unsigned long long n) { return !c->facts.known || n != 0ull || c->env_launch_all; }
-static unsigned list_grid(const l2r_ctx *c, uint32_t n) { return c->facts.known ? std::max(n, 1u) : (unsigned)std::max<int64_t>(c->n_tiles, 1); }
-
 static uint32_t *lc_this_run(const l2r_ctx *c) { return c->list_cnt.p + LC_WORDS * (c->lc_flip & 1u); }
 static uint32_t *lc_next_run(const l2r_ctx *c) { return c->list_cnt.p + LC_WORDS * ((c->lc_flip & 1u) ^ 1u); }
 static uint32_t *lc_last_run(const l2r_ctx *c) { return lc_next_run(c); }
@@ -431,7 +424,10 @@
             (e = hipEventCreateWithFlags(&c->ev_join[k], hipEventDisableTiming)) != hipSuccess) {
             fail(-2, "[l2r_create] side stream: %s", hipGetErrorString(e)); l2r_destroy(c); return nullptr;
         }
-    if ((e = hipEventCreateWithFlags(&c->ev_fork, hipEventDisableTiming)) != hipSuccess) { fail(-2, "[l2r_create] hipEventCreate: %s", hipGetErrorString(e)); l2r_destroy(c); return nullptr; }
+    if ((e = hipEventCreateWithFlags(&c->ev_fork, hipEventDisableTiming)) != hipSuccess || (e = hipEventCreateWithFlags(&c->ev_front, hipEventDisableTiming)) != hipSuccess) {
+        fail(-2, "[l2r_create] hipEventCreate: %s", hipGetErrorString(e)); l2r_destroy(c); return nullptr;
+    }
+    if ((e = hipHostMalloc((void **)&c->h_front, LC_WORDS * sizeof(uint32_t), hipHostMallocDefault)) != hipSuccess) { c->h_front = nullptr; fail(-2, "[l2r_create] hipHostMalloc: %s", hipGetErrorString(e)); l2r_destroy(c); return nullptr; }
     c->prm = l2r_params{3, 3, 50, 0, 0x7fffffff, 5, 0, 0, 1, 0, 0.80f};
     {
         hipDeviceProp_t prop;
@@ -456,6 +452,8 @@
         if (e) c->tile_split = atoi(e) != 0;
         e = getenv("L2R_SIDE");
         if (e) c->side_on = atoi(e) != 0;
+        e = getenv("L2R_FRONT_COUNTS");
+        if (e) c->front_on = atoi(e) != 0;
         c->env_stamps = getenv("L2R_STAMPS") != nullptr;
         e = getenv("L2R_PIPELINE");
         if (e) { c->want_pipe = !strcmp(e, "classic") ? Pipeline::classic : !strcmp(e, "slab") ? Pipeline::slab : Pipeline::tile; c->pipeline_forced = true; }
@@ -475,6 +473,8 @@
     (void)hipSetDevice(c->device);
     for (int k = 0; k < 2; ++k) { if (c->side[k]) (void)hipStreamDestroy(c->side[k]); if (c->ev_join[k]) (void)hipEventDestroy(c->ev_join[k]); }
     if (c->ev_fork) (void)hipEventDestroy(c->ev_fork);
+    if (c->ev_front) (void)hipEventDestroy(c->ev_front);
+    if (c->h_front) (void)hipHostFree(c->h_front);
     if (c->stream) (void)hipStreamDestroy(c->stream);
     delete c;
 }
@@ -815,16 +815,7 @@
     return fa;
 }
 
-static bool split_wait_free(const l2r_ctx *c) { return c->inexact_tiles == 0 && !(c->ablate & 256); }
-static uint32_t split_mode(const l2r_ctx *c)
-{
-    if (!c->tile_split || !c->rest_list.p) return SPLIT_OFF;
-    const uint32_t fits = (uint32_t)std::min<int64_t>((int64_t)c->n_cu * 4, c->tile_resident / 2);
-    if (c->facts.known) return c->facts.n_rest <= fits ? SPLIT_ON : SPLIT_OFF;
-    return split_wait_free(c) ? SPLIT_ON : SPLIT_LIST;
-}
-
-static SlabArgs slab_args(const l2r_ctx *c, const FastArgs &fa, const CursorDir &cd, bool tile)
+static SlabArgs slab_args(const l2r_ctx *c, const FastArgs &fa, const CursorDir &cd, bool tile, uint32_t split)
 {
     SlabArgs sa;
     sa.g.f = fa; sa.g.cd = cd; sa.g.tid_base = c->tid_base.p; sa.g.n_tid_dir = c->n_tid_dir; sa.g.tile_total = c->tile_total.p;
@@ -846,9 +837,11 @@
     sa.wide_direct_on = (tile && c->wide_direct && c->tw64.p && !(c->ablate & 4)) ? 1u : 0u;
     sa.chunk_direct_on = (tile && c->chunk_direct && sa.chunk_on) ? 1u : 0u;
     sa.rest_list = c->rest_list.p;
-    sa.split_on = tile ? split_mode(c) : SPLIT_OFF;
+    sa.split_on = tile ? split : SPLIT_OFF;
     return sa;
 }
+
+static void note_launch(l2r_ctx *c, unsigned grid) { c->n_launches++; c->n_workgroups += grid; }
 
 static void launch_probe(const l2r_ctx *c, const DevParams &p, const SlabArgs &sa, bool list, bool acc, unsigned grid)
 {
@@ -871,6 +864,7 @@
 {
     hipStream_t s = c->stream;
     const unsigned gt = (unsigned)(c->n_tiles ? c->n_tiles : 1);
+    note_launch(c, gt);
     with_flag(c->wide_cigar, [&](auto W) {
         hipLaunchKernelGGL(HIP_KERNEL_NAME(k_pass_a<W>), dim3(gt), dim3(TILE_THREADS), W ? pass_a_dynamic_lds(c->reads_per_tile) : 0, s, c->n_reads, c->r_tid.p, c->r_pos.p,
                            c->cig_off.p, c->cig.p, cd, tabs, p, (c->sorted ? (const int32_t *)nullptr : (const int32_t *)c->win_start.p), c->j0.p, c->local.p, c->order.p,
@@ -880,10 +874,12 @@
     {
         ScanJobs jobs = {}; jobs.job[0] = ScanJob{c->tile_base.p, c->n_tiles, c->totals.p + TOT_EXONS}; jobs.job[1] = jobs.job[0];
         hipLaunchKernelGGL(k_scan_u32, dim3(1), dim3(1024), 0, s, jobs);
+        note_launch(c, 1u);
     }
     MARK(ST_FAST);
     unsigned gp = (unsigned)std::min<int64_t>(c->n_tiles ? c->n_tiles : 1, (int64_t)c->n_cu * c->wg_per_cu);
     if (c->fast_grid > 0) gp = (unsigned)std::min<int64_t>(gp, c->fast_grid);
+    note_launch(c, gp);
     with_level(p.full_level, [&](auto L) { with_flag(c->wide_cigar, [&](auto W) {
         hipLaunchKernelGGL(HIP_KERNEL_NAME(k_classify_fast<L, W>), dim3(gp), dim3(TILE_THREADS), 0, s, fa, c->n_tiles, (const TileDesc *)c->desc.p,
                            (const uint32_t *)c->tile_base.p, (const int64_t *)c->cig_off.p, (const uint8_t *)c->order.p, (const uint32_t *)c->tile_first.p);
@@ -895,6 +891,7 @@
 {
     hipStream_t s = c->stream;
     const unsigned gx = 8u * (unsigned)std::max<int64_t>((c->n_tiles + 7) / 8, 1);
+    note_launch(c, gx);
     if (c->wide_cigar)
         hipLaunchKernelGGL(k_walk_slab_long, dim3(gx), dim3(TILE_THREADS), pass_a_dynamic_lds(c->reads_per_tile), s, sa, (const TileRec *)c->tile_rec.p);
     else
@@ -907,75 +904,115 @@
             HIP_TRY(hipMemcpyAsync(c->tile_xbase.p, c->tile_total.p, (size_t)c->n_tiles * 4, hipMemcpyDeviceToDevice, s));
             ScanJobs jobs = {}; jobs.job[0] = ScanJob{c->tile_xbase.p, c->n_tiles, c->totals.p + TOT_EXONS}; jobs.job[1] = jobs.job[0];
             hipLaunchKernelGGL(k_scan_u32, dim3(1), dim3(1024), 0, s, jobs);
+            note_launch(c, 1u);
             n_scan = 0;
         }
         const unsigned gd = n_scan + (unsigned)std::max<int64_t>((c->n_tiles + DESCRIBE_TILES - 1) / DESCRIBE_TILES, 1);
+        note_launch(c, gd);
         hipLaunchKernelGGL(HIP_KERNEL_NAME(k_describe_scan<false>), dim3(gd), dim3(TILE_THREADS), 0, s, sa, job, (uint32_t)n_scan, (const TileRec *)nullptr);
     }
     MARK(ST_FAST);
+    note_launch(c, gx);
     launch_probe(c, p, sa, false, (c->want & L2R_WANT_ACCEPTED) && c->n_sj == 0, gx);
     return 0;
 }
 
-static int launch_tile(l2r_ctx *c, hipEvent_t *ev, const DevParams &p, const SlabArgs &sa, bool skip_lists)
+static PlanIn plan_in(const l2r_ctx *c, bool events)
+{
+    PlanIn in;
+    in.pipeline = c->pipe == Pipeline::tile ? PLAN_TILE : c->pipe == Pipeline::slab ? PLAN_SLAB : PLAN_CLASSIC;
+    const bool tile = in.pipeline == PLAN_TILE;
+    in.facts = c->facts; in.front = c->front;
+    in.front_on = c->front_on; in.launch_all = c->env_launch_all; in.tile_split = c->tile_split && c->rest_list.p; in.side_on = c->side_on;
+    in.events_or_check = events || c->check_stages;
+    in.chunk_on = !(c->ablate & 32);
+    in.wide_direct_on = tile && c->wide_direct && c->tw64.p && !(c->ablate & 4);
+    in.chunk_direct_on = tile && c->chunk_direct && in.chunk_on;
+    in.no_exact_marks = (c->ablate & 256) != 0; in.sj_in_tail = (c->ablate & (512 | 1024)) != 0; in.has_wide_keys = c->n_wide > 0;
+    in.n_tiles = c->n_tiles; in.n_tiles256 = c->n_tiles256; in.seg_max = c->seg_max;
+    in.n_cu = c->n_cu; in.tile_resident = c->tile_resident;
+    in.inexact_tiles = c->inexact_tiles;
+    in.n_sj = c->n_sj; in.want_accepted = (c->want & L2R_WANT_ACCEPTED) != 0;
+    in.front_state = front_counts_apply(in) ? (c->front.known ? FRONT_CACHED : FRONT_PENDING) : FRONT_NONE;
+    return in;
+}
+static const Launch *plan_next(l2r_ctx *c, int kind)
+{
+    if (c->plan_at < c->plan.launches.size() && c->plan.launches[c->plan_at].kind == kind) return &c->plan.launches[c->plan_at++];
+    return nullptr;
+}
+
+static int launch_tile(l2r_ctx *c, hipEvent_t *ev, const DevParams &p, const SlabArgs &sa, PlanIn &in)
 {
     hipStream_t s = c->stream;
-    const RunFacts &f = c->facts;
     const DescribeScan job{c->tile_total.p, c->tile_xbase.p, c->totals.p + TOT_EXONS, c->n_tiles};
-    const unsigned gd = (unsigned)std::max<int64_t>((c->n_tiles + DESCRIBE_TILES - 1) / DESCRIBE_TILES, 1);
-    hipLaunchKernelGGL(HIP_KERNEL_NAME(k_describe_scan<true>), dim3(gd), dim3(TILE_THREADS), 0, s, sa, job, 0u, (const TileRec *)c->tile_rec.p);
-    MARK(ST_SCAN1);
-    const bool split = sa.split_on == SPLIT_ON;
-    const bool rest_launch = split && list_runs(c, f.n_rest);
-    const bool wide_launch = !skip_lists && sa.wide_direct_on && list_runs(c, f.n_wide);
-    const bool chunk_launch = !skip_lists && sa.chunk_direct_on && list_runs(c, f.n_chunk);
-    const bool beside = c->side_on && !ev && !c->check_stages;
-    const bool rest_side = rest_launch && beside && split_wait_free(c);
-    const bool wide_side = wide_launch && beside, chunk_side = chunk_launch && beside;
-    const bool side0 = rest_side || wide_side, side1 = chunk_side;
-    const unsigned gf = fused_grid(c->n_tiles), gr = list_grid(c, f.n_rest), gwd = list_grid(c, f.n_wide), gcd = list_grid(c, f.n_chunk);
-    if (rest_launch && !rest_side) launch_k_tile<false, false>(c, p, sa, gr, s);
-    if (side0 || side1) HIP_TRY(hipEventRecord(c->ev_fork, s));
-    if (side0) HIP_TRY(hipStreamWaitEvent(c->side[0], c->ev_fork, 0));
-    if (rest_side) launch_k_tile<false, false>(c, p, sa, gr, c->side[0]);
-    if (wide_launch) launch_k_tile<true, false>(c, p, sa, gwd, wide_side ? c->side[0] : s);
-    if (side0) HIP_TRY(hipEventRecord(c->ev_join[0], c->side[0]));
-    if (side1) {
-        HIP_TRY(hipStreamWaitEvent(c->side[1], c->ev_fork, 0));
-        launch_tile_chunk(c, p, sa, gcd, 0u, c->side[1]);
-        HIP_TRY(hipEventRecord(c->ev_join[1], c->side[1]));
-    }
-    if (split) launch_k_tile<false, true>(c, p, sa, gf, s);
-    else launch_k_tile<false, false>(c, p, sa, gf, s);
-    MARK(ST_FAST);
-    if (chunk_launch && !chunk_side) launch_tile_chunk(c, p, sa, gcd, 0u, s);
-    if (side0) HIP_TRY(hipStreamWaitEvent(s, c->ev_join[0], 0));
-    if (side1) HIP_TRY(hipStreamWaitEvent(s, c->ev_join[1], 0));
-    const unsigned gl = (unsigned)std::min<int64_t>(c->n_tiles ? c->n_tiles : 1, (int64_t)c->n_cu * 2);
-    if (!skip_lists && list_runs(c, f.n_fb)) launch_probe(c, p, sa, true, false, gl);
-    return 0;
-}
-
-static void launch_lists(l2r_ctx *c, const DevParams &p, const SlabArgs &sa, bool tile, bool skip_lists)
-{
-    if (skip_lists) return;
+    bool forked = false, waits[2] = {false, false}, used[2] = {false, false};
+    for (; c->plan_at < c->plan.launches.size() && c->plan.launches[c->plan_at].kind <= LK_TILE_CHUNK; ++c->plan_at) {
+        const Launch l = c->plan.launches[c->plan_at];
+        hipStream_t st = s;
+        if (l.stream != LS_MAIN) {
+            const int k = l.stream == LS_SIDE0 ? 0 : 1;
+            if (!forked) { HIP_TRY(hipEventRecord(c->ev_fork, s)); forked = true; }
+            if (!waits[k]) { HIP_TRY(hipStreamWaitEvent(c->side[k], c->ev_fork, 0)); waits[k] = true; }
+            used[k] = used[k] || launch_is_kernel(l.kind);
+            st = c->side[k];
+        }
+        if (launch_is_kernel(l.kind)) note_launch(c, l.grid);
+        switch (l.kind) {
+        case LK_DESCRIBE:
+            hipLaunchKernelGGL(HIP_KERNEL_NAME(k_describe_scan<true>), dim3(l.grid), dim3(TILE_THREADS), 0, st, sa, job, 0u, (const TileRec *)c->tile_rec.p);
+            MARK(ST_SCAN1);
+            break;
+        case LK_FRONT_COPY:
+            HIP_TRY(hipMemcpyAsync(c->h_front, lc_this_run(c), LC_WORDS * sizeof(uint32_t), hipMemcpyDeviceToHost, st));
+            HIP_TRY(hipEventRecord(c->ev_front, st));
+            break;
+        case LK_TILE_GENERAL: launch_k_tile<false, false>(c, p, sa, l.grid, st); MARK(ST_FAST); break;
+        case LK_TILE_EXACT: launch_k_tile<false, true>(c, p, sa, l.grid, st); MARK(ST_FAST); break;
+        case LK_FRONT_WAIT: {
+            HIP_TRY(hipEventSynchronize(c->ev_front));
+            c->front.known = true; c->front.n_wide = c->h_front[LC_WIDE]; c->front.n_chunk = c->h_front[LC_CHUNK]; c->front.n_rest = c->h_front[LC_REST];
+            in.front = c->front; in.front_state = FRONT_READ;
+            LaunchPlan next = launch_plan(in);
+            bool same = next.split == c->plan.split && next.launches.size() > c->plan_at;
+            for (size_t i = 0; same && i <= c->plan_at; ++i) {
+                const Launch &x = next.launches[i], &y = c->plan.launches[i];
+                same = x.kind == y.kind && x.grid == y.grid && x.stream == y.stream && x.place == y.place;
+            }
+            if (!same) return fail(-2, "[launch_tile] the launch plan changed in front of the wait for the front counts");
+            c->plan = std::move(next);
+            break; }
+        case LK_TILE_REST: launch_k_tile<false, false>(c, p, sa, l.grid, st); break;
+        case LK_TILE_WIDE: launch_k_tile<true, false>(c, p, sa, l.grid, st); break;
+        case LK_TILE_CHUNK: launch_tile_chunk(c, p, sa, l.grid, 0u, st); break;
+        default: break;
+        }
+    }
+    for (int k = 0; k < 2; ++k)
+        if (used[k]) { HIP_TRY(hipEventRecord(c->ev_join[k], c->side[k])); HIP_TRY(hipStreamWaitEvent(s, c->ev_join[k], 0)); }
+    if (const Launch *l = plan_next(c, LK_PROBE_LIST)) { note_launch(c, l->grid); launch_probe(c, p, sa, true, false, l->grid); }
+    return 0;
+}
+
+static void launch_lists(l2r_ctx *c, const DevParams &p, const SlabArgs &sa, bool tile)
+{
     hipStream_t s = c->stream;
-    const RunFacts &f = c->facts;
-    if (!tile || list_runs(c, f.n_wide_rest)) {
+    if (const Launch *l = plan_next(c, LK_PROBE_WIDE)) {
         const WideArgs wa{c->tw64.p};
-        const unsigned gw = (unsigned)std::min<int64_t>(c->n_tiles ? c->n_tiles : 1, (int64_t)c->n_cu * 5);
+        note_launch(c, l->grid);
         with_level(p.full_level, [&](auto L) {
-            hipLaunchKernelGGL(HIP_KERNEL_NAME(k_probe_slab_wide<L>), dim3(gw), dim3(TILE_THREADS), 0, s, sa, wa, (const uint32_t *)c->tile_first.p, (const int32_t *)c->r_pos.p,
+            hipLaunchKernelGGL(HIP_KERNEL_NAME(k_probe_slab_wide<L>), dim3(l->grid), dim3(TILE_THREADS), 0, s, sa, wa, (const uint32_t *)c->tile_first.p, (const int32_t *)c->r_pos.p,
                                (const uint32_t *)c->tile_sbase.p, (const TileWin *)c->tw.p, (const uint32_t *)c->tile_xbase.p, (const TileStat *)(tile ? c->tile_stat.p : nullptr));
         });
     }
-    if (sa.chunk_direct_on && list_runs(c, f.n_late)) {
-        launch_tile_chunk(c, p, sa, list_grid(c, f.n_late), 1u, s);
-    }
-    if (sa.chunk_on && (!tile || list_runs(c, f.chunk_rest))) {
-        const unsigned gc = (unsigned)std::min<int64_t>(c->n_tiles ? c->n_tiles : 1, (int64_t)c->n_cu * 4);
+    if (const Launch *l = plan_next(c, LK_TILE_CHUNK_LATE)) {
+        note_launch(c, l->grid);
+        launch_tile_chunk(c, p, sa, l->grid, 1u, s);
+    }
+    if (const Launch *l = plan_next(c, LK_PROBE_CHUNKED)) {
+        note_launch(c, l->grid);
         with_level(p.full_level, [&](auto L) {
-            hipLaunchKernelGGL(HIP_KERNEL_NAME(k_probe_slab_chunked<L>), dim3(gc), dim3(TILE_THREADS), 0, s, sa, (const uint32_t *)c->tile_first.p, (const int32_t *)c->r_pos.p,
+            hipLaunchKernelGGL(HIP_KERNEL_NAME(k_probe_slab_chunked<L>), dim3(l->grid), dim3(TILE_THREADS), 0, s, sa, (const uint32_t *)c->tile_first.p, (const int32_t *)c->r_pos.p,
                                (const uint32_t *)c->tile_sbase.p, (const TileWin *)c->tw.p, (const uint32_t *)c->tile_xbase.p);
         });
     }
@@ -985,47 +1022,48 @@
 {
     hipStream_t s = c->stream;
     const bool tile = c->pipe == Pipeline::tile;
-    const unsigned gt = (unsigned)(c->n_tiles ? c->n_tiles : 1), g256 = (unsigned)(c->n_tiles256 ? c->n_tiles256 : 1);
     MARK(ST_GENERIC);
-    const bool sj_left = c->n_sj > 0 && (c->ablate & (512 | 1024)) != 0;
-    const bool nothing_left = tile && c->facts.known && c->facts.redo_empty && (lists_empty(c->facts) || c->n_sj == 0) && !c->env_launch_all && !sj_left;
     end_of_run(c, tile);
-    if (!nothing_left) {
-        const unsigned gg = (unsigned)std::min<int64_t>(c->n_tiles ? c->n_tiles * 4 : 1, 4096);
-        hipLaunchKernelGGL(k_classify_generic, dim3(gg), dim3(TILE_THREADS), 0, s, c->totals.p + TOT_REDO, c->redo.p, c->r_tid.p, c->r_rev.p,
+    if (const Launch *l = plan_next(c, LK_GENERIC)) {
+        note_launch(c, l->grid);
+        hipLaunchKernelGGL(k_classify_generic, dim3(l->grid), dim3(TILE_THREADS), 0, s, c->totals.p + TOT_REDO, c->redo.p, c->r_tid.p, c->r_rev.p,
                            (c->pipe != Pipeline::classic ? (const int32_t *)nullptr : j0),
                            c->hdr.p, c->anno_ex.p, p, c->ex_off.p, c->ex_start.p, c->ex_end.p, c->ex_flag.p, c->info.p, c->ref_tx.p,
                            c->tile_acc.p, c->tile_acc_ex.p, (const uint32_t *)c->tile_first.p, (int)c->n_tiles, cd);
     }
     MARK(ST_SJ);
-    if (c->n_sj > 0 && !nothing_left) {
+    if (const Launch *l = plan_next(c, LK_VALIDATE_SJ)) {
         if (!c->sorted) { int rc = prepare_unsorted_sj_cursor(c); if (rc) return rc; }
-        hipLaunchKernelGGL(k_validate_sj, dim3(g256), dim3(TILE_THREADS), 0, s, c->n_reads, c->r_tid.p, c->ex_off.p, c->ex_start.p, c->ex_end.p, c->ex_flag.p,
+        note_launch(c, l->grid);
+        hipLaunchKernelGGL(k_validate_sj, dim3(l->grid), dim3(TILE_THREADS), 0, s, c->n_reads, c->r_tid.p, c->ex_off.p, c->ex_start.p, c->ex_end.p, c->ex_flag.p,
                            c->sj_key.p, (c->sorted ? (const int32_t *)nullptr : c->sj_cursor.p), c->sj_tid.p, c->sj_don.p, c->sj_acc.p,
                            c->sj_uniq.p, c->sj_multi.p, p, c->info.p,
                            SjDir{CursorDir{c->sj_key.p, c->sj_cdir.p, c->sj_cbase.p, c->sj_ntid, (int32_t)c->n_sj}, c->sj_ddir.p, c->sj_dbase.p, c->sj_ntid, c->sj_row.p});
     }
-    if ((c->n_sj > 0 || c->pipe != Pipeline::classic) && (c->want & L2R_WANT_ACCEPTED)) {
-        hipLaunchKernelGGL(k_count_accepted, dim3((gt + 3u) / 4u), dim3(TILE_THREADS), 0, s, (const uint32_t *)c->tile_first.p, c->info.p, (const uint32_t *)c->tile_chunk.p, c->tile_acc.p, c->tile_acc_ex.p, (uint32_t)c->n_tiles);
+    if (const Launch *l = plan_next(c, LK_COUNT_ACCEPTED)) {
+        note_launch(c, l->grid);
+        hipLaunchKernelGGL(k_count_accepted, dim3(l->grid), dim3(TILE_THREADS), 0, s, (const uint32_t *)c->tile_first.p, c->info.p, (const uint32_t *)c->tile_chunk.p, c->tile_acc.p, c->tile_acc_ex.p, (uint32_t)c->n_tiles);
     }
     MARK(ST_SCAN2);
-    if (c->want & L2R_WANT_ACCEPTED) {
+    if (const Launch *l = plan_next(c, LK_SCAN_ACCEPTED)) {
+        note_launch(c, l->grid);
         if (c->n_tiles <= c->seg_max) {
-            const unsigned n_seg = (unsigned)std::max<int64_t>((c->n_tiles + SEG_COUNT - 1) / SEG_COUNT, 1);
-            hipLaunchKernelGGL(k_scan_segments, dim3(2u * n_seg), dim3(TILE_THREADS), 0, s, SegScan{c->tile_acc.p, c->tile_acc_at.p, c->totals.p + TOT_ACCEPTED, c->n_tiles},
-                               SegScan{c->tile_acc_ex.p, c->tile_acc_ex_at.p, c->totals.p + TOT_ACCEPTED_EXONS, c->n_tiles}, (uint32_t)n_seg);
+            hipLaunchKernelGGL(k_scan_segments, dim3(l->grid), dim3(TILE_THREADS), 0, s, SegScan{c->tile_acc.p, c->tile_acc_at.p, c->totals.p + TOT_ACCEPTED, c->n_tiles},
+                               SegScan{c->tile_acc_ex.p, c->tile_acc_ex_at.p, c->totals.p + TOT_ACCEPTED_EXONS, c->n_tiles}, (uint32_t)(l->grid / 2u));
         } else {
             HIP_TRY(hipMemcpyAsync(c->tile_acc_at.p, c->tile_acc.p, (size_t)c->n_tiles * 4, hipMemcpyDeviceToDevice, s));
             HIP_TRY(hipMemcpyAsync(c->tile_acc_ex_at.p, c->tile_acc_ex.p, (size_t)c->n_tiles * 4, hipMemcpyDeviceToDevice, s));
             ScanJobs jobs = {}; jobs.job[0] = ScanJob{c->tile_acc_at.p, c->n_tiles, c->totals.p + TOT_ACCEPTED}; jobs.job[1] = ScanJob{c->tile_acc_ex_at.p, c->n_tiles, c->totals.p + TOT_ACCEPTED_EXONS};
-            hipLaunchKernelGGL(k_scan_u32, dim3(2), dim3(1024), 0, s, jobs);
+            hipLaunchKernelGGL(k_scan_u32, dim3(l->grid), dim3(1024), 0, s, jobs);
         }
     }
     MARK(ST_GATHER);
-    if (c->want & L2R_WANT_ACCEPTED)
-        hipLaunchKernelGGL(k_gather_accepted, dim3((gt + GATHER_TILES - 1) / GATHER_TILES), dim3(TILE_THREADS), 0, s, (const uint32_t *)c->tile_first.p, c->first_read, c->info.p, c->ref_tx.p, c->ex_off.p,
+    if (const Launch *l = plan_next(c, LK_GATHER_ACCEPTED)) {
+        note_launch(c, l->grid);
+        hipLaunchKernelGGL(k_gather_accepted, dim3(l->grid), dim3(TILE_THREADS), 0, s, (const uint32_t *)c->tile_first.p, c->first_read, c->info.p, c->ref_tx.p, c->ex_off.p,
                            c->ex_start.p, c->ex_end.p, c->ex_flag.p, c->tile_acc_at.p, c->tile_acc_ex_at.p, c->tile_chunk.p, c->tile_rchunk.p, c->totals.p + TOT_CHUNK_CURSOR,
                            c->acc_rec.p, c->acc_ex_off.p, c->acc_start.p, c->acc_end.p, c->acc_flag.p, (uint32_t)c->n_tiles);
+    }
     MARK(ST_N);
     return 0;
 }
@@ -1035,6 +1073,9 @@
     const DevParams p = dev_params(c);
     MARK(ST_PASS_A);
     c->pipe = choose_pipeline(c, p);
+    PlanIn in = plan_in(c, ev != nullptr);
+    c->plan = launch_plan(in); c->plan_at = 0;
+    c->n_launches = 0; c->n_workgroups = 0; c->front_used = FRONT_NONE;
     const int32_t *j0 = c->sorted ? (const int32_t *)c->j0.p : (const int32_t *)c->win_start.p;
     const CursorDir cd{c->anno_key.p, c->key_dir.p, c->kb_base.p, c->n_tid_key, (int32_t)c->n_tx};
     const SiteTabs tabs{{c->sk_st.p, c->sd_st.p, c->sr_st.p}, {c->sk_en.p, c->sd_en.p, nullptr}, c->tid_base.p, c->n_tid_dir};
@@ -1044,13 +1085,13 @@
     else {
         const bool tile = c->pipe == Pipeline::tile;
         if (tile && !c->prev_run_tile) HIP_TRY(lc_reset(c));
-        const SlabArgs sa = slab_args(c, fa, cd, tile);
-        const bool skip_lists = tile && c->facts.known && lists_empty(c->facts) && !c->env_launch_all;
-        rc = tile ? launch_tile(c, ev, p, sa, skip_lists) : launch_slab(c, ev, p, sa);
-        if (!rc) launch_lists(c, p, sa, tile, skip_lists);
+        const SlabArgs sa = slab_args(c, fa, cd, tile, c->plan.split);
+        rc = tile ? launch_tile(c, ev, p, sa, in) : launch_slab(c, ev, p, sa);
+        if (!rc) launch_lists(c, p, sa, tile);
     }
     if (!rc) rc = launch_tail(c, ev, p, cd, j0);
     if (rc) return rc;
+    c->front_used = c->plan.front;
     HIP_TRY(hipGetLastError());
     return 0;
 }
@@ -1095,6 +1136,7 @@
     if (n >= 12) for (int k = 0; k < 8; ++k) out[4 + k] = 0;
     if (n >= 13) out[12] = 0;
     for (int k = 16; k < std::min(n, 29); ++k) out[k] = 0;
+    if (n >= 32) { out[29] = c->n_launches; out[30] = c->n_workgroups; out[31] = c->front_used; }
     if (n >= 14) out[13] = c->n_lb_fallback;
     if (n >= 16) {
         out[14] = 0; out[15] = 0;
diff --git a/lr2rmats_amd/csrc/l2r_launchplan.hip.h b/lr2rmats_amd/csrc/l2r_launchplan.hip.h
--- /dev/null
+++ b/lr2rmats_amd/csrc/l2r_launchplan.hip.h
@@ -0,0 +1,160 @@
+#pragma once
+#include <assert.h>
+#include <stdint.h>
+#include <algorithm>
+#include <vector>
+
+namespace l2r {
+
+struct RunFacts {
+    bool known = false;
+    uint32_t n_wide = 0;
+    uint32_t n_chunk = 0;
+    uint32_t n_rest = 0;
+    uint32_t n_late = 0;
+    uint32_t n_fb = 0;
+    uint32_t n_wide_rest = 0;
+    unsigned long long chunk_rest = 0;
+    bool redo_empty = false;
+};
+
+struct FrontCounts {
+    bool known = false;
+    uint32_t n_wide = 0, n_chunk = 0, n_rest = 0;
+};
+enum { FRONT_NONE = 0, FRONT_READ = 1, FRONT_CACHED = 2, FRONT_PENDING = 3 };
+
+enum { PLAN_CLASSIC = 0, PLAN_SLAB = 1, PLAN_TILE = 2 };
+
+struct PlanIn {
+    int pipeline = PLAN_TILE;
+    RunFacts facts;
+    FrontCounts front; int front_state = FRONT_NONE;
+    bool front_on = true;
+    bool launch_all = false;
+    bool tile_split = true;
+    bool side_on = true;
+    bool events_or_check = false;
+    bool wide_direct_on = true, chunk_direct_on = true, chunk_on = true;
+    bool no_exact_marks = false;
+    bool sj_in_tail = false;
+    bool has_wide_keys = false;
+    int64_t n_tiles = 0, n_tiles256 = 0, seg_max = 0;
+    int n_cu = 256; int64_t tile_resident = 0;
+    int64_t inexact_tiles = 0;
+    int64_t n_sj = 0;
+    bool want_accepted = false;
+};
+
+enum LaunchKind {
+    LK_DESCRIBE = 0,
+    LK_FRONT_COPY, LK_FRONT_WAIT,
+    LK_TILE_GENERAL,
+    LK_TILE_EXACT,
+    LK_TILE_REST,
+    LK_TILE_WIDE,
+    LK_TILE_CHUNK,
+    LK_PROBE_LIST,
+    LK_PROBE_WIDE,
+    LK_TILE_CHUNK_LATE,
+    LK_PROBE_CHUNKED,
+    LK_GENERIC, LK_VALIDATE_SJ, LK_COUNT_ACCEPTED, LK_SCAN_ACCEPTED, LK_GATHER_ACCEPTED,
+    LK_N
+};
+enum LaunchStream { LS_MAIN = 0, LS_SIDE0 = 1, LS_SIDE1 = 2 };
+enum LaunchPlace { LP_BEFORE = 0, LP_MAIN = 1, LP_BEHIND = 2 };
+inline bool launch_is_kernel(int kind) { return kind != LK_FRONT_COPY && kind != LK_FRONT_WAIT; }
+
+struct Launch { int kind; unsigned grid; int stream; int place; };
+struct LaunchPlan {
+    std::vector<Launch> launches;
+    uint32_t split = SPLIT_OFF;
+    int front = FRONT_NONE;
+    bool skip_lists = false;
+};
+
+inline bool lists_empty(const RunFacts &f) { return f.n_fb == 0u && f.n_wide == 0u && f.n_chunk == 0u && f.n_late == 0u; }
+
+inline bool split_wait_free(const PlanIn &in) { return in.inexact_tiles == 0 && !in.no_exact_marks; }
+inline uint32_t split_mode(const PlanIn &in)
+{
+    if (!in.tile_split) return SPLIT_OFF;
+    const uint32_t fits = (uint32_t)std::min<int64_t>((int64_t)in.n_cu * 4, in.tile_resident / 2);
+    if (in.facts.known) return in.facts.n_rest <= fits ? SPLIT_ON : SPLIT_OFF;
+    return split_wait_free(in) ? SPLIT_ON : SPLIT_LIST;
+}
+
+inline bool front_counts_apply(const PlanIn &in) { return in.pipeline == PLAN_TILE && in.front_on && !in.facts.known && !in.launch_all; }
+
+inline LaunchPlan launch_plan(const PlanIn &in)
+{
+    LaunchPlan pl;
+    std::vector<Launch> &L = pl.launches;
+    const RunFacts &f = in.facts;
+    const bool tile = in.pipeline == PLAN_TILE;
+    const int64_t nt = in.n_tiles;
+    const unsigned gt = (unsigned)std::max<int64_t>(nt, 1);
+    auto list_runs = [&](unsigned long long n) { return !f.known || n != 0ull || in.launch_all; };
+    auto list_grid = [&](uint32_t n) { return f.known ? std::max(n, 1u) : gt; };
+    const bool front = in.front_state != FRONT_NONE && front_counts_apply(in);
+    const bool counted = front && in.front_state != FRONT_PENDING;
+    const FrontCounts &fc = in.front;
+    pl.front = front ? in.front_state : FRONT_NONE;
+    pl.split = tile ? split_mode(in) : SPLIT_OFF;
+    const bool split = pl.split == SPLIT_ON;
+    pl.skip_lists = tile && f.known && lists_empty(f) && !in.launch_all;
+    const bool none_listed = counted && split && fc.n_wide == 0u && fc.n_chunk == 0u && fc.n_rest == 0u;
+    if (none_listed) pl.skip_lists = true;
+    const uint64_t late_bound = std::min<uint64_t>((uint64_t)std::max<int64_t>(nt, 0), (split ? (uint64_t)fc.n_rest : (uint64_t)std::max<int64_t>(nt, 0)) + fc.n_wide);
+
+    if (tile) {
+        L.push_back({LK_DESCRIBE, (unsigned)std::max<int64_t>((nt + DESCRIBE_TILES - 1) / DESCRIBE_TILES, 1), LS_MAIN, LP_BEFORE});
+        const bool beside = in.side_on && !in.events_or_check;
+        const unsigned gf = fused_grid(nt);
+        const Launch main_instance{split ? LK_TILE_EXACT : LK_TILE_GENERAL, gf, LS_MAIN, LP_MAIN};
+        if (!front) {
+            const bool rest_launch = split && list_runs(f.n_rest);
+            const bool wide_launch = !pl.skip_lists && in.wide_direct_on && list_runs(f.n_wide);
+            const bool chunk_launch = !pl.skip_lists && in.chunk_direct_on && list_runs(f.n_chunk);
+            const bool rest_side = rest_launch && beside && split_wait_free(in);
+            if (rest_launch) L.push_back({LK_TILE_REST, list_grid(f.n_rest), rest_side ? LS_SIDE0 : LS_MAIN, LP_BEFORE});
+            if (wide_launch) L.push_back({LK_TILE_WIDE, list_grid(f.n_wide), beside ? LS_SIDE0 : LS_MAIN, LP_BEFORE});
+            if (chunk_launch && beside) L.push_back({LK_TILE_CHUNK, list_grid(f.n_chunk), LS_SIDE1, LP_BEFORE});
+            L.push_back(main_instance);
+            if (chunk_launch && !beside) L.push_back({LK_TILE_CHUNK, list_grid(f.n_chunk), LS_MAIN, LP_BEHIND});
+        } else {
+            assert(!split || split_wait_free(in));
+            const bool rest_is_all = split && in.has_wide_keys && nt > 0;
+            if (in.front_state != FRONT_CACHED) L.push_back({LK_FRONT_COPY, 0u, beside ? (rest_is_all ? LS_SIDE1 : LS_SIDE0) : LS_MAIN, LP_BEFORE});
+            L.push_back(main_instance);
+            if (rest_is_all) L.push_back({LK_TILE_REST, gt, beside ? LS_SIDE0 : LS_MAIN, LP_BEHIND});
+            if (in.front_state != FRONT_CACHED) L.push_back({LK_FRONT_WAIT, 0u, LS_MAIN, LP_BEHIND});
+            if (!counted) return pl;
+            if (split && fc.n_rest != 0u && !rest_is_all) L.push_back({LK_TILE_REST, fc.n_rest, beside ? LS_SIDE0 : LS_MAIN, LP_BEHIND});
+            if (in.wide_direct_on && fc.n_wide != 0u) L.push_back({LK_TILE_WIDE, fc.n_wide, beside ? LS_SIDE0 : LS_MAIN, LP_BEHIND});
+            if (in.chunk_direct_on && fc.n_chunk != 0u) L.push_back({LK_TILE_CHUNK, fc.n_chunk, beside ? LS_SIDE1 : LS_MAIN, LP_BEHIND});
+        }
+        if (!pl.skip_lists && list_runs(f.n_fb)) L.push_back({LK_PROBE_LIST, (unsigned)std::min<int64_t>(gt, (int64_t)in.n_cu * 2), LS_MAIN, LP_BEHIND});
+        for (const Launch &l : L) { assert(!(front && l.place == LP_BEFORE && launch_is_kernel(l.kind) && l.kind != LK_DESCRIBE)); (void)l; }
+    }
+    if (in.pipeline != PLAN_CLASSIC && !pl.skip_lists) {
+        if (!tile || list_runs(f.n_wide_rest)) L.push_back({LK_PROBE_WIDE, (unsigned)std::min<int64_t>(gt, (int64_t)in.n_cu * 5), LS_MAIN, LP_BEHIND});
+        if (tile && in.chunk_direct_on && list_runs(f.n_late)) {
+            if (!counted) L.push_back({LK_TILE_CHUNK_LATE, list_grid(f.n_late), LS_MAIN, LP_BEHIND});
+            else if (late_bound != 0u) L.push_back({LK_TILE_CHUNK_LATE, (unsigned)late_bound, LS_MAIN, LP_BEHIND});
+        }
+        if (in.chunk_on && (!tile || list_runs(f.chunk_rest))) L.push_back({LK_PROBE_CHUNKED, (unsigned)std::min<int64_t>(gt, (int64_t)in.n_cu * 4), LS_MAIN, LP_BEHIND});
+    }
+    const bool sj_left = in.n_sj > 0 && in.sj_in_tail;
+    const bool nothing_left = tile && f.known && f.redo_empty && (lists_empty(f) || in.n_sj == 0) && !in.launch_all && !sj_left;
+    if (!nothing_left) L.push_back({LK_GENERIC, (unsigned)std::min<int64_t>(nt ? nt * 4 : 1, 4096), LS_MAIN, LP_BEHIND});
+    if (in.n_sj > 0 && !nothing_left) L.push_back({LK_VALIDATE_SJ, (unsigned)std::max<int64_t>(in.n_tiles256, 1), LS_MAIN, LP_BEHIND});
+    if (in.want_accepted) {
+        if (in.n_sj > 0 || in.pipeline != PLAN_CLASSIC) L.push_back({LK_COUNT_ACCEPTED, (gt + 3u) / 4u, LS_MAIN, LP_BEHIND});
+        L.push_back({LK_SCAN_ACCEPTED, nt <= in.seg_max ? 2u * (unsigned)std::max<int64_t>((nt + SEG_COUNT - 1) / SEG_COUNT, 1) : 2u, LS_MAIN, LP_BEHIND});
+        L.push_back({LK_GATHER_ACCEPTED, (gt + (unsigned)GATHER_TILES - 1u) / (unsigned)GATHER_TILES, LS_MAIN, LP_BEHIND});
+    }
+    return pl;
+}
+
+}
```

After: 23.22 billion (median of 2 runs). No clear change (+0.6%).
